# JuliaGenAI/ColBERT.jl

Measured on AMD Instinct MI355X. Metric: queries/sec, top-1000 on 1M-passage corpus, higher is better.
Workload: dtype f32

## Files before the change

colbert.jl_amd/csrc/approx_kernels.hpp:

```cpp
#pragma once
#include <hip/hip_fp16.h>

#include <algorithm>

#include "common.hpp"
#include "search_kernels.hpp"

namespace clb {

typedef __bf16 bf16x8 __attribute__((ext_vector_type(8)));
typedef uint32_t u32x4 __attribute__((ext_vector_type(4)));
typedef uint32_t u32x4_a4 __attribute__((ext_vector_type(4), aligned(4)));
typedef float f32x4_a4 __attribute__((ext_vector_type(4), aligned(4)));

constexpr float kEpsSafety = 1.25f;

inline bool approx_supported(int dim, int nbits) { return dim == kDim && nbits == 2; }
inline size_t approx_cells_bytes(int64_t B, int64_t K, int64_t ) { return (size_t)B * K * 16 * 4 + 2048; }

__device__ __forceinline__ uint32_t f32_to_bf16_rne(float f) {
    const uint32_t u = __float_as_uint(f);
    return (u + 0x7fffu + ((u >> 16) & 1u)) >> 16;
}
__device__ __forceinline__ uint32_t pack_bf16(float lo, float hi) {
// ... 769 lines not shown
            }
            topn_insert<2>(tv, ti, a, id);
        }
        }
    } else {
        for (int c = lane; c < K; c += 64) {
            const float* cr = C + (size_t)c * kDim;
            float a = 0.f;
            for (int d = 0; d < kDim; ++d) a = fmaf(cr[d], qs[d], a);
            topn_insert<2>(tv, ti, a, c);
        }
        if (lane == 0) atomicAdd(&redo_flag[b], 1);
    }
#pragma unroll
    for (int o = 32; o > 0; o >>= 1) {
        const float v0 = __shfl_xor(tv[0], o, 64), v1 = __shfl_xor(tv[1], o, 64);
        const int i0 = __shfl_xor(ti[0], o, 64), i1 = __shfl_xor(ti[1], o, 64);
        topn_insert<2>(tv, ti, v0, i0);
        topn_insert<2>(tv, ti, v1, i1);
    }
    if (lane == 0) {
        sel[((size_t)b * 32 + t) * 2] = ti[0];
        sel[((size_t)b * 32 + t) * 2 + 1] = ti[1] == 0x7fffffff ? ti[0] : ti[1];
    }
}

static __global__ __launch_bounds__(256) void cells_to_half_kernel(const float* __restrict__ cells,
                                                                  uint32_t* __restrict__ cells16, int K) {
    const int b = blockIdx.y;
    const float* src = cells + (size_t)b * K * 32;
    uint32_t* dst = cells16 + (size_t)b * K * 16;
    const int64_t total = (int64_t)K * 16;
    for (int64_t i = (int64_t)blockIdx.x * 256 + threadIdx.x; i < total; i += (int64_t)gridDim.x * 256) {
        const int64_t c = i >> 4;
        const int t = (int)(i & 15);
        const float lo = src[c * 32 + 2 * t], hi = src[c * 32 + 2 * t + 1];
        const __half2 h = __floats2half2_rn(lo, hi);
        dst[i] = *reinterpret_cast<const uint32_t*>(&h);
    }
}

typedef _Float16 f16x8 __attribute__((ext_vector_type(8)));

struct StepTag {
    int j;
    int rows;
    int last;
    int base;
    int g;
    int jh;
    int rowsh;
    int baseh;
};

constexpr int kStepRows = 32;
constexpr uint32_t kPackSpan = (1u << 27) - kStepRows;

__device__ __forceinline__ uint32_t f32_to_f16_floor(float x) {
    const __half hr = __float2half_rn(x);
    uint32_t bits = *reinterpret_cast<const uint16_t*>(&hr);
    if (__half2float(hr) > x) bits = (bits & 0x8000u) ? bits + 1u : (bits == 0u ? 0x8001u : bits - 1u);
    return bits;
}

template <int N>
__device__ __forceinline__ uint32_t lut_offset(uint32_t R, uint32_t lane8) {
    return __builtin_amdgcn_perm(R, lane8, 0x0c0c0000u | ((4u + N) << 8));
}

#define CLB_DPP_F(V, CTRL) __builtin_bit_cast(float, __builtin_amdgcn_update_dpp(0, __builtin_bit_cast(int, (V)), (CTRL), 0xf, 0xf, true))
__device__ __forceinline__ float sum_lanes_0_31(float s) {
    s += CLB_DPP_F(s, 0xB1);
    s += CLB_DPP_F(s, 0x4E);
    s += CLB_DPP_F(s, 0x141);
    s += CLB_DPP_F(s, 0x140);
    const float below = __builtin_bit_cast(float, __builtin_amdgcn_update_dpp(0, __builtin_bit_cast(int, s), 0x142, 0xa, 0xf, false));
    return s + below;
}
__device__ __forceinline__ float max_lane_halves(float m) { return fmaxf(m, __shfl_xor(m, 32, 64)); }

constexpr int kApproxThreads = 768;
constexpr int kApproxLdsLut = 256 * 256;

template <bool ROWS, int GL = 0, bool CELL8 = false>
static __global__ __launch_bounds__(kApproxThreads, kApproxThreads / 256) void score_approx32_kernel(
    const float* __restrict__ weights, const uint32_t* __restrict__ codeinv, const uint8_t* __restrict__ residuals,
    int cbits, float inv_lo, float inv_step, const float* __restrict__ Q, const uint32_t* __restrict__ cells16,
    const uint2* __restrict__ cand_hdr, const int* __restrict__ ncand, float* __restrict__ scores, int K, int T,
    int B, size_t cand_cap, uint16_t* __restrict__ tokmax, const int* __restrict__ list,
    const int* __restrict__ nlist, const float* __restrict__ eps_pair, unsigned long long* __restrict__ rowmask,
    const float4* __restrict__ tscale = nullptr) {
    const uint32_t cmask = (1u << cbits) - 1u;
    const int lane = threadIdx.x & 63;
    const int r = lane & 31, h = lane >> 5;
    const int x = blockIdx.x & 7;
    const int wg = blockIdx.x >> 3;
    const int wg_per_group = gridDim.x >> 3;
    const int wave = __builtin_amdgcn_readfirstlane(threadIdx.x >> 6);
    __shared__ __attribute__((aligned(16))) unsigned char lut_s[kApproxLdsLut];
    __shared__ __attribute__((aligned(16))) float invx[kApproxThreads / 64][2 * kStepRows];
    constexpr int kSlotBytes = CELL8 ? 1024 : 2048;
    constexpr int kRingBytes = 3 * kSlotBytes;
    __shared__ __attribute__((aligned(16))) unsigned char ring_s[GL ? (kApproxThreads / 64) * kRingBytes : 16];
    constexpr int kStageBytes = 16 * 64 + 64;
    __shared__ __attribute__((aligned(16))) unsigned char stage_s[ROWS ? 16 : (kApproxThreads / 64) * kStageBytes];
    unsigned char* mystage = stage_s + (ROWS ? 0 : wave * kStageBytes);
    __shared__ uint32_t mask_s[ROWS ? (kApproxThreads / 64) * 32 : 1];
    uint32_t* mymask = mask_s + (ROWS ? wave * 32 : 0);
    if (ROWS && threadIdx.x < (kApproxThreads / 64) * 32) mask_s[threadIdx.x] = 0u;
    for (int i = threadIdx.x; i < 256 * 32; i += kApproxThreads) {
        const int v = i >> 5;
        *reinterpret_cast<uint2*>(lut_s + (size_t)i * 8) =
            make_uint2(pack_f16(weights[v & 3], weights[(v >> 2) & 3]), pack_f16(weights[(v >> 4) & 3], weights[(v >> 6) & 3]));
    }
    __syncthreads();
    const char* lut = reinterpret_cast<const char*>(lut_s);
    float* myinv = invx[wave];
    const uint32_t lane8 = 8u * (uint32_t)r;
    unsigned char* myring = ring_s + (GL ? wave * kRingBytes : 0);
    const uint32_t ring_lds = (uint32_t)(uintptr_t)(__attribute__((address_space(3))) unsigned char*)myring;
    const uint32_t gl_poff = 16u * (((uint32_t)lane - (((uint32_t)lane >> 4) & 3u)) & 3u);
    const int gl_src0 = (int)((uint32_t)lane & ~3u);
    const int gl_src1 = gl_src0 + 64;
    const uint32_t gl_rot = ((uint32_t)r >> 2) & 3u;
    const uint32_t gl_x0 = (uint32_t)r * 64u + 16u * (((uint32_t)h + gl_rot) & 3u);
    const uint32_t gl_x1 = (uint32_t)r * 64u + 16u * (((uint32_t)h + 2u + gl_rot) & 3u);
    const int gl8_src = (int)(((uint32_t)lane >> 1) << 2);
    const uint32_t gl8_poff = 16u * (((uint32_t)lane ^ ((uint32_t)lane >> 4)) & 1u);
    const uint32_t gl8_x = (uint32_t)r * 32u + 16u * (((uint32_t)h ^ ((uint32_t)r >> 3)) & 1u);

    f16x8 sel1, sel2;
#pragma unroll
    for (int j = 0; j < 8; ++j) {
        sel1[j] = (r == (CELL8 ? 16 * h + j : 8 * h + j)) ? (_Float16)1.0f : (_Float16)0.0f;
        sel2[j] = (r == (CELL8 ? 16 * h + 8 + j : 16 + 8 * h + j)) ? (_Float16)1.0f : (_Float16)0.0f;
    }

    int b_first, b_step, sub, nsub;
    if (B >= 8) { b_first = x; b_step = 8; sub = 0; nsub = 1; }
    else { b_first = x % B; b_step = B * 8 ; sub = x / B; nsub = (8 - b_first + B - 1) / B; }
    const bool grid2d = gridDim.y > 1;
    const int wg_count = grid2d ? (int)gridDim.x : wg_per_group;
    const int wg_index = grid2d ? (int)blockIdx.x : wg;
    if (grid2d) { b_first = blockIdx.y; b_step = B; sub = 0; nsub = 1; }

    for (int b = b_first; b < B; b += b_step) {
        u32x4 qb[8];
        const float4 ts = CELL8 ? tscale[(size_t)b * 32 + r] : make_float4(1.f, 1.f, 0.f, 0.f);
        const float stp = ts.x;
        const float acc_init = CELL8 ? ts.z - 1024.0f : 0.f;
        {
            const float* qrow = Q + ((size_t)b * T + (r < T ? r : T - 1)) * kDim + 64 * h;
#pragma unroll
            for (int s = 0; s < 8; ++s) {
                float4 lo = *reinterpret_cast<const float4*>(qrow + 8 * s);
                float4 hi = *reinterpret_cast<const float4*>(qrow + 8 * s + 4);
                if (r >= T) { lo = make_float4(0.f, 0.f, 0.f, 0.f); hi = lo; }
                if (CELL8) {
                    lo.x *= ts.y; lo.y *= ts.y; lo.z *= ts.y; lo.w *= ts.y;
                    hi.x *= ts.y; hi.y *= ts.y; hi.z *= ts.y; hi.w *= ts.y;
                }
                qb[s] = u32x4{pack_f16(lo.x, lo.y), pack_f16(lo.z, lo.w), pack_f16(hi.x, hi.y), pack_f16(hi.z, hi.w)};
            }
        }
        const uint2* hdr = cand_hdr + (size_t)b * cand_cap;
        const char* c16 = reinterpret_cast<const char*>(cells16 + (size_t)b * K * (CELL8 ? 8 : 16));
        const uint32_t h16 = 16u * (uint32_t)h;
        float* out = scores + (size_t)b * cand_cap;
        uint16_t* tmax = tokmax + (size_t)b * cand_cap * 32 + r;
        const int* lst = ROWS ? list + (size_t)b * cand_cap : nullptr;
        unsigned long long* rmask = ROWS ? rowmask + (size_t)b * cand_cap * 8 : nullptr;
        const float window = ROWS ? 2.f * eps_pair[b] : 0.f;
        const int n = ROWS ? nlist[b] : ncand[b];
        const int n_waves = wg_count * (kApproxThreads / 64) * nsub;
        const int my_wave = (sub * wg_count + wg_index) * (kApproxThreads / 64) + wave;
        const int per_wave = (n + n_waves - 1) / n_waves;
        const int j_first = min(n, my_wave * per_wave), j_end = min(n, j_first + per_wave);

        for (int j0 = j_first; j0 < j_end; j0 += 64) {
        const int jl = j0 + lane;
        int slot_l = jl < j_end ? jl : j0;
        if (ROWS) slot_l = lst[slot_l];
        const uint2 hv = hdr[slot_l];
        const int nd = j_end - j0 < 64 ? j_end - j0 : 64;
        int it_k = 0;
        uint32_t it_off = __builtin_amdgcn_readlane(hv.x, 0);
        int it_len = (int)__builtin_amdgcn_readlane(hv.y, 0);
        int it_slot = __builtin_amdgcn_readlane(slot_l, 0);
        int it_base = 0;

#define CLB_STAGE_A(RB, CV, PM, TAG)                                                                    \
    {                                                                                                       \
        const bool live = it_k < nd;                                                                        \
        const uint32_t e0 = live ? it_off + (uint32_t)it_base : 0u;                                         \
        const int left = live ? it_len - it_base : kStepRows;                                               \
        const int rows = left < kStepRows ? left : kStepRows;                                               \
        int slot_t = live ? it_slot : 0;                                                                    \
        uint32_t d_ = 0;                                                                                    \
        TAG.j = live ? j0 + it_k : -1;                                                                      \
        TAG.rows = rows;                                                                                    \
        TAG.last = 0;                                                                                       \
        TAG.base = it_base;                                                                                 \
        TAG.g = 0; TAG.jh = -1; TAG.rowsh = rows; TAG.baseh = 0;                                            \
        if (left <= kStepRows) {                                        \
            const int kb = it_k + 1;                                                                        \
            const int kk = kb < 64 ? kb : 63;                                                               \
            const uint32_t off_b = __builtin_amdgcn_readlane(hv.x, kk);                                     \
            const int len_b = (int)__builtin_amdgcn_readlane(hv.y, kk);                                     \
            const int slot_b = __builtin_amdgcn_readlane(slot_l, kk);                                       \
            const int gq = (rows + 7) >> 3;                                                                 \
            d_ = off_b - e0;                     \
            if (!ROWS && gq >= 1 && gq < 4 && kb < nd && len_b > 0 && d_ < kPackSpan) {    \
                const int cap = kStepRows - 8 * gq;                                                         \
                TAG.g = gq; TAG.jh = TAG.j; TAG.rowsh = rows; TAG.baseh = it_base;                          \
                TAG.j = j0 + kb; TAG.rows = len_b < cap ? len_b : cap; TAG.base = 0;                         \
                slot_t = slot_b;                                                                            \
                if (len_b <= cap) {                                           \
                    TAG.last = kb + 1 >= nd ? 3 : 1;                                                        \
                    it_k = kb + 1;                                                                          \
                    const int kc = it_k < 64 ? it_k : 63;                                                   \
                    it_off = __builtin_amdgcn_readlane(hv.x, kc);                                           \
                    it_len = (int)__builtin_amdgcn_readlane(hv.y, kc);                                      \
                    it_slot = __builtin_amdgcn_readlane(slot_l, kc);                                        \
                    it_base = 0;                                                                            \
                } else {                                                                                    \
                    it_k = kb; it_off = off_b; it_len = len_b; it_slot = slot_b; it_base = cap;             \
                }                                                                                           \
            } else {                                                                                        \
                d_ = 0;                                                                                     \
                TAG.last = kb >= nd ? 3 : 1;                                                                \
                it_k = kb; it_off = off_b; it_len = len_b; it_slot = slot_b; it_base = 0;                   \
            }                                                                                               \
        } else it_base += kStepRows;                                                                        \
        if (ROWS) PM = tmax[(size_t)slot_t * 32];               \
        const uint32_t q8_ = 8u * (uint32_t)TAG.g;                                                          \
                       \
        const uint32_t rr = (uint32_t)r < q8_ ? min((uint32_t)r, (uint32_t)(TAG.rowsh - 1))                 \
                                              : min((uint32_t)r, q8_ + (uint32_t)(TAG.rows - 1)) + (d_ - q8_); \
         \
        const uint8_t* rbase_ = residuals + (size_t)e0 * 32;                                                \
        const char* cbase_ = reinterpret_cast<const char*>(codeinv + (size_t)e0);                           \
        const uint32_t roff_ = rr * 32u + h16;                                                              \
        const uint32_t coff_ = rr * 4u;                                                                     \
         \
         \
        RB = __builtin_nontemporal_load(reinterpret_cast<const u32x4*>(rbase_ + roff_));                    \
        CV = __builtin_nontemporal_load(reinterpret_cast<const uint32_t*>(cbase_ + coff_));    \
    }
#define CLB_STAGE_G(CV, X0, X1, SLOT)                                                                       \
    if (GL && CELL8) {                                                                                      \
        const uint32_t ca_ = (uint32_t)__builtin_amdgcn_ds_bpermute(gl8_src, (int)CV) & cmask;              \
        asm volatile("s_mov_b32 m0, %1\n\tglobal_load_lds_dwordx4 %0, off"                                  \
                     :: "v"(c16 + ((ca_ << 5) + gl8_poff)), "s"(ring_lds + (SLOT) * 1024u) : "memory");     \
    } else if (GL) {                                                                                        \
        const uint32_t ca_ = (uint32_t)__builtin_amdgcn_ds_bpermute(gl_src0, (int)CV) & cmask;              \
        const uint32_t cb_ = (uint32_t)__builtin_amdgcn_ds_bpermute(gl_src1, (int)CV) & cmask;              \
         \
        asm volatile("s_mov_b32 m0, %2\n\tglobal_load_lds_dwordx4 %0, off\n\t"                            \
                     "s_add_u32 m0, m0, 0x400\n\tglobal_load_lds_dwordx4 %1, off"                          \
                     :: "v"(c16 + ((ca_ << 6) + gl_poff)), "v"(c16 + ((cb_ << 6) + gl_poff)),               \
                        "s"(ring_lds + (SLOT) * 2048u) : "memory", "scc");                                   \
    } else {                                                                                                \
        const char* row_ = CELL8 ? c16 + (((CV & cmask) << 5) + h16) : c16 + (((CV & cmask) << 6) + h16);   \
        if (CELL8) X0 = *reinterpret_cast<const u32x4*>(row_);       \
        else {                                                                                              \
        X0 = *reinterpret_cast<const u32x4*>(row_);                                                         \
        X1 = *reinterpret_cast<const u32x4*>(row_ + 32);                                                    \
        }                                                                                                   \
    }
#define CLB_LUT(W, N) (*reinterpret_cast<const uint2*>(lut + lut_offset<N>(W, lane8)))
#define CLB_STAGE_CM(RB, CV, X0, X1, SLOT, ACC)                                                       \
    {                                                                                                       \
        if (GL && CELL8) {                                                                                  \
             \
            asm volatile("s_waitcnt vmcnt(3)" ::: "memory");                                                \
            X0 = *reinterpret_cast<const u32x4*>(myring + (SLOT) * 1024 + gl8_x);                           \
        } else if (GL) {                                                                                    \
             \
            asm volatile("s_waitcnt vmcnt(4)" ::: "memory");                                                \
            X0 = *reinterpret_cast<const u32x4*>(myring + (SLOT) * 2048 + gl_x0);                           \
            X1 = *reinterpret_cast<const u32x4*>(myring + (SLOT) * 2048 + gl_x1);                           \
        }                                                                                                   \
         \
        __builtin_amdgcn_wave_barrier();                                                                    \
        myinv[r] = fmaf((float)(CV >> cbits), inv_step, inv_lo);                                            \
        __builtin_amdgcn_wave_barrier();                                                                    \
         \
         \
         \
        uint2 tl[16];                                                                                       \
        tl[0] = CLB_LUT(RB[0], 0); tl[1] = CLB_LUT(RB[0], 1); tl[2] = CLB_LUT(RB[0], 2); tl[3] = CLB_LUT(RB[0], 3);         \
        tl[4] = CLB_LUT(RB[1], 0); tl[5] = CLB_LUT(RB[1], 1); tl[6] = CLB_LUT(RB[1], 2); tl[7] = CLB_LUT(RB[1], 3);         \
        tl[8] = CLB_LUT(RB[2], 0); tl[9] = CLB_LUT(RB[2], 1); tl[10] = CLB_LUT(RB[2], 2); tl[11] = CLB_LUT(RB[2], 3);       \
        tl[12] = CLB_LUT(RB[3], 0); tl[13] = CLB_LUT(RB[3], 1); tl[14] = CLB_LUT(RB[3], 2); tl[15] = CLB_LUT(RB[3], 3);     \
        __builtin_amdgcn_sched_barrier(0);                                                                  \
        _Pragma("unroll") for (int i = 0; i < 16; ++i) ACC[i] = acc_init;                                   \
        if (CELL8) {                     \
            const u32x4 raw_ = X0;                                                                          \
            X0 = u32x4{__builtin_amdgcn_perm(0x64646464u, raw_[0], 0x04010400u), __builtin_amdgcn_perm(0x64646464u, raw_[0], 0x04030402u), \
                       __builtin_amdgcn_perm(0x64646464u, raw_[1], 0x04010400u), __builtin_amdgcn_perm(0x64646464u, raw_[1], 0x04030402u)}; \
            X1 = u32x4{__builtin_amdgcn_perm(0x64646464u, raw_[2], 0x04010400u), __builtin_amdgcn_perm(0x64646464u, raw_[2], 0x04030402u), \
                       __builtin_amdgcn_perm(0x64646464u, raw_[3], 0x04010400u), __builtin_amdgcn_perm(0x64646464u, raw_[3], 0x04030402u)}; \
        }                                                                                                   \
        ACC = __builtin_amdgcn_mfma_f32_32x32x16_f16(__builtin_bit_cast(f16x8, X0), sel1, ACC, 0, 0, 0);    \
        ACC = __builtin_amdgcn_mfma_f32_32x32x16_f16(__builtin_bit_cast(f16x8, X1), sel2, ACC, 0, 0, 0);    \
        _Pragma("unroll") for (int s_ = 0; s_ < 8; ++s_)                                                    \
            ACC = __builtin_amdgcn_mfma_f32_32x32x16_f16(                                                   \
                __builtin_bit_cast(f16x8, u32x4{tl[2 * s_].x, tl[2 * s_].y, tl[2 * s_ + 1].x, tl[2 * s_ + 1].y}), \
                __builtin_bit_cast(f16x8, qb[s_]), ACC, 0, 0, 0);                                           \
    }
#define CLB_PASSAGE_END(MX, J, LAST)                                                                        \
    {                                                                                                       \
        float m_ = max_lane_halves(MX);                                                                     \
        if (CELL8) m_ *= stp;                         \
        const float sum = sum_lanes_0_31(r < T ? m_ : 0.f);                      \
        if ((J) >= 0) {                                                                                \
                   \
            const int p_ = ((J) - j0) & 15;                                                                 \
            if (h == 0) *reinterpret_cast<uint16_t*>(mystage + p_ * 64 + 2 * r) = (uint16_t)f32_to_f16_floor(m_); \
            if (lane == 16) *reinterpret_cast<float*>(mystage + 1024 + 4 * p_) = sum;                       \
            if (p_ == 15 || (LAST) == 3) {     \
                const int jb_ = (J) - p_;                                                                   \
                __builtin_amdgcn_wave_barrier();                                                            \
                const u32x4 tk_ = *reinterpret_cast<const u32x4*>(mystage + 16 * lane);                     \
                const float sc_ = *reinterpret_cast<const float*>(mystage + 1024 + 4 * (lane & 15));         \
                if (lane < 4 * (p_ + 1))                                                                    \
                    *reinterpret_cast<u32x4*>(reinterpret_cast<unsigned char*>(tokmax + ((size_t)b * cand_cap + jb_) * 32) + 16 * lane) = tk_; \
                if (lane <= p_) out[jb_ + lane] = sc_;                                                      \
                __builtin_amdgcn_wave_barrier();                                                            \
            }                                                                                               \
        }                                                                                                   \
    }
#define CLB_STAGE_E(ACC, PM, TAG)                                                                     \
    {                                                                                                       \
        f32x4 iq[4];                                                                                        \
        _Pragma("unroll") for (int q = 0; q < 4; ++q)                                                       \
            iq[q] = *reinterpret_cast<const f32x4*>(myinv + 8 * q + 4 * h);                                 \
         \
         \
         \
        float v[16];                                                                                        \
        _Pragma("unroll") for (int i = 0; i < 16; ++i) { v[i] = ACC[i] * iq[i >> 2][i & 3]; asm volatile("" : "+v"(v[i])); } \
        if (ROWS) {                                                                                         \
            const __half pmh = *reinterpret_cast<const __half*>(&PM);                                       \
            const float lo = r < T ? __half2float(pmh) - window : __builtin_inff();    \
             \
             \
             \
            uint32_t lm = 0;                                                                                \
            _Pragma("unroll") for (int i = 0; i < 16; ++i) lm |= !((CELL8 ? v[i] * stp : v[i]) < lo) ? (1u << i) : 0u; \
            lm |= (uint32_t)__builtin_amdgcn_update_dpp(0, (int)lm, 0xB1, 0xf, 0xf, true);         \
            lm |= (uint32_t)__builtin_amdgcn_update_dpp(0, (int)lm, 0x4E, 0xf, 0xf, true);         \
            lm |= (uint32_t)__builtin_amdgcn_update_dpp(0, (int)lm, 0x141, 0xf, 0xf, true);    \
            lm |= (uint32_t)__builtin_amdgcn_update_dpp(0, (int)lm, 0x140, 0xf, 0xf, true);      \
             \
             \
             \
             \
            uint32_t sp_ = ((lm & 0xFu) | ((lm & 0xF0u) << 4) | ((lm & 0xF00u) << 8) | ((lm & 0xF000u) << 12)) << (4 * h); \
            sp_ &= TAG.rows < kStepRows ? (1u << TAG.rows) - 1u : 0xffffffffu;                              \
             \
             \
             \
             \
             \
            const int wd_ = TAG.base >> 5;                                                                  \
            int ln_ = lane;                                                                                 \
            asm volatile("" : "+v"(ln_));      \
            if ((ln_ & 15) == 0 && wd_ < 8 && TAG.j >= 0) mymask[wd_ + 8 * (((ln_ >> 3) & 2) | (ln_ >> 5))] = sp_; \
            if (TAG.last) {                                                                                 \
                __builtin_amdgcn_wave_barrier();                                                            \
                if (ln_ < 16) {          \
                    const int d_ = (ln_ & 7) + 16 * (ln_ >> 3);                                             \
                    const uint32_t mv_ = mymask[d_] | mymask[d_ + 8];                                       \
                    if (TAG.j >= 0) reinterpret_cast<uint32_t*>(rmask + (size_t)TAG.j * 8)[ln_] = mv_;      \
                    mymask[d_] = 0u;                                                                        \
                    mymask[d_ + 8] = 0u;                                                                    \
                }                                                                                           \
                __builtin_amdgcn_wave_barrier();                                                            \
            }                                                                                               \
        } else {                                                                                            \
            if (TAG.g) {               \
                const float q0_ = fmaxf(fmaxf(fmaxf(v[0], v[1]), v[2]), v[3]);                              \
                const float q1_ = fmaxf(fmaxf(fmaxf(v[4], v[5]), v[6]), v[7]);                              \
                const float q2_ = fmaxf(fmaxf(fmaxf(v[8], v[9]), v[10]), v[11]);                            \
                const float q3_ = fmaxf(fmaxf(fmaxf(v[12], v[13]), v[14]), v[15]);                          \
                const float mh_ = fmaxf(fmaxf(mx, q0_), fmaxf(TAG.g > 1 ? q1_ : kNegInf, TAG.g > 2 ? q2_ : kNegInf)); \
                CLB_PASSAGE_END(mh_, TAG.jh, 1);                                                            \
                mx = fmaxf(fmaxf(TAG.g > 1 ? kNegInf : q1_, TAG.g > 2 ? kNegInf : q2_), q3_);               \
            } else {                                                                                        \
            float m01 = fmaxf(fmaxf(v[0], v[1]), v[2]);                                                     \
            float m23 = fmaxf(fmaxf(v[3], v[4]), v[5]);                                                     \
            float m45 = fmaxf(fmaxf(v[6], v[7]), v[8]);                                                     \
            float m67 = fmaxf(fmaxf(v[9], v[10]), v[11]);                                                   \
            float m89 = fmaxf(fmaxf(v[12], v[13]), v[14]);                                                  \
            m01 = fmaxf(fmaxf(m01, m23), m45);                                                              \
            m67 = fmaxf(fmaxf(m67, m89), v[15]);                                                            \
            mx = fmaxf(fmaxf(mx, m01), m67);                                                                \
            }                                                                                               \
            if (TAG.last) {                                                                                 \
                CLB_PASSAGE_END(mx, TAG.j, TAG.last);                                                       \
                mx = kNegInf;                                                                               \
            }                                                                                               \
        }                                                                                                   \
    }

        float mx = kNegInf;
        u32x4 rb0, rb1, rb2, xa0, xa1, xa2, xb0, xb1, xb2;
        uint32_t cv0, cv1, cv2, cw0, cw1, cw2;
        uint16_t pm0 = 0, pm1 = 0, pm2 = 0;
        StepTag t0, t1, t2;
        f32x16 acc0;
        CLB_STAGE_A(rb0, cv0, pm0, t0);
        CLB_STAGE_A(rb1, cv1, pm1, t1);
        CLB_STAGE_G(cv0, xa0, xb0, 0); cw0 = cv0;
        while (t0.j >= 0) {
            CLB_STAGE_A(rb2, cv2, pm2, t2);
            CLB_STAGE_G(cv1, xa1, xb1, 1); cw1 = cv1;
            CLB_STAGE_CM(rb0, cw0, xa0, xb0, 0, acc0);
            CLB_STAGE_E(acc0, pm0, t0);
            CLB_STAGE_A(rb0, cv0, pm0, t0);
            CLB_STAGE_G(cv2, xa2, xb2, 2); cw2 = cv2;
            CLB_STAGE_CM(rb1, cw1, xa1, xb1, 1, acc0);
            CLB_STAGE_E(acc0, pm1, t1);
            CLB_STAGE_A(rb1, cv1, pm1, t1);
            CLB_STAGE_G(cv0, xa0, xb0, 0); cw0 = cv0;
            CLB_STAGE_CM(rb2, cw2, xa2, xb2, 2, acc0);
            CLB_STAGE_E(acc0, pm2, t2);
        }
        }
#undef CLB_STAGE_A
#undef CLB_STAGE_G
#undef CLB_STAGE_CM
#undef CLB_STAGE_E
#undef CLB_PASSAGE_END
#undef CLB_LUT
    }
}

static __global__ __launch_bounds__(256) void code_adjacency_kernel(const uint32_t* __restrict__ codes0, int64_t n,
                                                                   unsigned long long* __restrict__ count) {
    unsigned long long c = 0;
    for (int64_t i = (int64_t)blockIdx.x * 256 + threadIdx.x + 1; i < n; i += (int64_t)gridDim.x * 256)
        c += (codes0[i] >> 1) == (codes0[i - 1] >> 1);
#pragma unroll
    for (int o = 32; o > 0; o >>= 1) c += __shfl_xor(c, o, 64);
    if ((threadIdx.x & 63) == 0 && c) atomicAdd(count, c);
}

struct ApproxConsts {
    float cn_max;
    float rn_max;
    float inv_max;
    float rb_max;
    float dw_rn;
    float inv_qerr;
    float dc_max;
};

struct QueryBound { float eps_t, eps_sum; bool unsafe; };
__device__ __forceinline__ QueryBound query_bound(const float* __restrict__ Q, int b, int T, const ApproxConsts& ac,
                                                  float* s_qn, float* s_dq, const float4* __restrict__ tscale = nullptr,
                                                  float* s_aux = nullptr ,
                                                  bool cell8 = false) {
    const int tid = threadIdx.x;
    if (tid == 0) { *s_qn = 0.f; *s_dq = 0.f; }
    if (tscale && tid < 4) s_aux[tid] = 0.f;
    __syncthreads();
    {
        const int t = tid >> 5, part = tid & 31;
        float a = 0.f, dd = 0.f, d8 = 0.f;
        if (t < T) {
            const float4 v = *reinterpret_cast<const float4*>(Q + ((size_t)b * T + t) * kDim + 4 * part);
            a = fmaf(v.x, v.x, fmaf(v.y, v.y, fmaf(v.z, v.z, v.w * v.w)));
            const float dx = v.x - round_f16(v.x), dy = v.y - round_f16(v.y);
            const float dz = v.z - round_f16(v.z), dw = v.w - round_f16(v.w);
            dd = fmaf(dx, dx, fmaf(dy, dy, fmaf(dz, dz, dw * dw)));
            if (tscale && cell8) {
                const float4 ts = tscale[(size_t)b * 32 + t];
                const float sx = v.x * ts.y, sy = v.y * ts.y, sz = v.z * ts.y, sw = v.w * ts.y;
                const float ex = sx - round_f16(sx), ey = sy - round_f16(sy), ez = sz - round_f16(sz), ew = sw - round_f16(sw);
                d8 = fmaf(ex, ex, fmaf(ey, ey, fmaf(ez, ez, ew * ew)));
            }
        }
#pragma unroll
        for (int o = 16; o > 0; o >>= 1) { a += __shfl_xor(a, o, 64); dd += __shfl_xor(dd, o, 64); d8 += __shfl_xor(d8, o, 64); }
        if (t < T && part == 0) {
            atomicMax(reinterpret_cast<unsigned int*>(s_qn), __float_as_uint(sqrtf(a) * 1.001f));
            atomicMax(reinterpret_cast<unsigned int*>(s_dq), __float_as_uint(sqrtf(dd) * 1.001f));
            if (tscale) {
                const float4 ts = tscale[(size_t)b * 32 + t];
                atomicMax(reinterpret_cast<unsigned int*>(s_aux), __float_as_uint(ts.x * sqrtf(d8) * 1.001f));
                atomicMax(reinterpret_cast<unsigned int*>(s_aux + 1), __float_as_uint(ts.x));
                atomicMax(reinterpret_cast<unsigned int*>(s_aux + 3), __float_as_uint(ts.w));
                if (!(ts.x > 0.f) || !(sqrtf(a) * ts.y < 3.0e4f)) s_aux[2] = 1.f;
            }
        }
    }
    __syncthreads();
    const float u = 5.9604645e-08f;
    const float qn = *s_qn;
    const float e_cells = kEpsSafety * centroid_product_bound(qn, *s_dq, ac.cn_max, ac.dc_max) + 4.8828125e-04f * qn * ac.cn_max + 2.9802322e-08f;
    float e_qr = 1.001f * (*s_dq * ac.rb_max + qn * ac.dw_rn) + 2.f * 128.f * u * qn * ac.rn_max;
    float e_tab = e_cells;
    bool bad8 = false;
    if (tscale) {
        const float amax = s_aux[2] != 0.f ? qn * ac.cn_max : fminf(s_aux[3] * 1.0001f, qn * ac.cn_max);
        const float e_f16 = kEpsSafety * centroid_product_bound(qn, *s_dq, ac.cn_max, ac.dc_max) + 4.8828125e-04f * amax + 2.9802322e-08f;
        e_tab = e_f16;
        if (cell8) {
            const float dq8 = s_aux[0], step_max = s_aux[1];
// ... 472 lines not shown
```

colbert.jl_amd/csrc/search.hip:

```cpp
#include <algorithm>
#include <atomic>
#include <cstdlib>
#include <cstring>
#include <memory>
#include <numeric>

#include "approx_kernels.hpp"
#include "after_kernels.hpp"
#include "generic_kernels.hpp"
#include "group_kernels.hpp"
#include "index_change_kernels.hpp"
#include "prior_kernels.hpp"
#include "search_kernels.hpp"
#include "sort.hpp"

using namespace clb;

namespace {

enum KernelId {
    KID_CENTROID_SCORES = 0,
    KID_TOPN,
    KID_MARK,
    KID_COMPACT,
    KID_SCORE_EXACT,
    KID_SCORE_APPROX,
    KID_SELECT,
    KID_ROWS,
    KID_TOPK,
    KID_COUNT
};
const char* kKernelNames[KID_COUNT] = {"centroid_scores", "top_nprobe", "mark_candidates", "compact_candidates",
                                       "score_exact",     "score_approx", "select_margin", "rescore_rows",
                                       "topk"};

struct Prof {
    bool on = false;
    bool counters = false;
    std::vector<std::pair<hipEvent_t, hipEvent_t>> pending[KID_COUNT];
    std::vector<hipEvent_t> pool;
    hipEvent_t chain = nullptr;
    hipStream_t chain_stream = nullptr;
    double total_ms[KID_COUNT] = {0};
    int64_t launches[KID_COUNT] = {0};
    bool failed = false;
    hipEvent_t get() {
        if (!pool.empty()) {
            hipEvent_t e = pool.back();
            pool.pop_back();
            return e;
        }
        hipEvent_t e = nullptr;
        if (hipEventCreate(&e) != hipSuccess) { failed = true; return nullptr; }
        return e;
    }
};

}

struct clb_filter {
    uint64_t owner = 0;
    int device = 0;
    int64_t n_docs = 0, count = 0;
    DevBuf bits;
};

struct clb_grouping {
    uint64_t owner = 0;
    int device = 0;
    int64_t n_docs = 0, count = 0;
    DevBuf gid;
};

struct clb_prior {
    uint64_t owner = 0;
    int device = 0;
    int64_t n_docs = 0;
    float max_abs = 0.f;
    DevBuf values;
};

struct Workspace {
    int64_t Bcap = 0, Tcap = 0, npcap = 0, kcap = 0;
    int64_t Ttuned = 0;
    size_t cand_cap = 0;
    int W = 0, nblk_bitmap = 0, topn_blocks = 0;
    bool x1_table = false;
    bool have_range = false;
    bool cell8 = false;
    size_t filt_cap = 0;
    size_t ivf_cap = 0;
    struct { bool valid = false; const float* dQ = nullptr; int64_t T = 0, B = 0, nprobe = 0, k = 0; void* stream = nullptr;
             size_t filt_now = 0; const clb_grouping* grp = nullptr; int64_t group_base = 0;
             const clb_prior* prior = nullptr; float weight = 0.f; } pending;
    struct { bool valid = false; int64_t B = 0, k = 0, generation = 0; const clb_grouping* grp = nullptr; void* stream = nullptr; } grouped_done;
    DevBuf Qdev, cells, cells_q, partial, sel, bitmap, blocksum, ncand, cand, cand_hdr, scores, list, nlist, thresh,
        outp, outs, flags, stats, redo, rowmask, eps_pair, tokmax, tau_glob, wsel, bounds, tscale, rangep, cells8;
    bool grouped = false;
    DevBuf grp_list, grp_n, grp_list2, grp_n2, grp_tau;
    int64_t mcap = 0;
    DevBuf hit_p, hit_s, hit_cut, hit_run, hit_list, hit_n;
    bool prior = false;
    DevBuf prior_tau;
    bool after = false;
    DevBuf after_list, after_n, after_tau, after_cur_s, after_cur_p;
    DevBuf g_cells, g_keys, g_keys2, g_vals, g_vals2, g_scratch, g_sort_tmp;
};

constexpr int kWorkspaceSlots = 4;

struct clb_searcher {
    int device = 0;
    uint64_t serial = 0;
    int64_t dim = 0, K = 0, n_docs = 0, n_emb = 0, pid_offset = 0;
    int nbits = 0;
    int mode = 0;
    int wide_select = -1;
    bool approx_ok = false;
    bool bounds_synced = false;
    bool ivf_sorted = false;
    bool generic = false;
    int64_t max_doclen = 0;
    hipStream_t stream = nullptr;
    DevBuf centroids;
    DevBuf weights;
    DevBuf codes0;
    DevBuf residuals;
    DevBuf doc_off;
    DevBuf live;
    DevBuf ivf_off;
    DevBuf ivf_pid;
    DevBuf codeinv;
    int cbits = 0;
    float inv_lo = 0.f, inv_step = 0.f;
    DevBuf cent_hi, cent_lo;
    DevBuf cent_f16;
    float dc_f16 = 0.f;
    int s1_x1 = -1;
    int gather_lds = 0;
    double code_adjacency = 0.0;
    int cell8 = -1;
    ApproxConsts approx_consts{};
    std::vector<uint32_t> ivf_len_sorted;
    Workspace ws[kWorkspaceSlots];
    Prof prof;
    int64_t last_cand_docs = 0, last_cand_embs = 0, last_resc_docs = 0, last_resc_embs = 0;
    int64_t index_bytes = 0;
    int64_t generation = 0;
};

namespace {

struct Batch {
    const float* dQ = nullptr;
    int B = 0, T = 0, nprobe = 0, k = 0;
    int64_t* d_out_pids = nullptr; float* d_out_scores = nullptr; int64_t* d_n_cand = nullptr;
    const clb_filter* const* filt = nullptr;
    int filt_all = 0;
    size_t filt_now = 0;
    const clb_grouping* grp = nullptr;
    int per_group = 0;
    int64_t* d_hit_pids = nullptr; float* d_hit_scores = nullptr;
    const clb_prior* prior = nullptr;
    float prior_weight = 1.f;
    const float* d_after_s = nullptr; const int64_t* d_after_p = nullptr;
    bool stats_keep = false;
    int phase = 0, n_shards = 0;
    float* d_local_top = nullptr; const float* d_all_top = nullptr;
    int64_t group_base = 0;
    int64_t* d_local_gid = nullptr; const int64_t* d_all_gid = nullptr;
    int64_t* d_out_gids = nullptr; int64_t* d_edge_gids = nullptr;
    float* d_local_mabs = nullptr; const float* d_all_mabs = nullptr;
};
Batch make_batch(const float* dQ, int64_t B, int64_t T, int64_t nprobe, int64_t k) {
    Batch q;
    q.dQ = dQ; q.B = (int)B; q.T = (int)T; q.nprobe = (int)nprobe; q.k = (int)k;
    return q;
}

struct Timed {
    clb_searcher* s;
    int id;
    hipStream_t st;
    hipEvent_t a = nullptr, b = nullptr;
    Timed(clb_searcher* s_, int id_, hipStream_t st_) : s(s_), id(id_), st(st_) {
        if (s->prof.on && id >= 0) {
            if (s->prof.chain && s->prof.chain_stream == st) {
                a = s->prof.chain;
            } else {
                a = s->prof.get();
                if (a && hipEventRecord(a, st) != hipSuccess) { s->prof.pool.push_back(a); a = nullptr; s->prof.failed = true; }
            }
            b = a ? s->prof.get() : nullptr;
        }
    }
    ~Timed() {
        if (!s->prof.on || id < 0) return;
        if (a && b && hipEventRecord(b, st) == hipSuccess) {
            s->prof.pending[id].push_back({a, b});
            s->prof.chain = b;
            s->prof.chain_stream = st;
        } else {
            s->prof.failed = true;
            s->prof.chain = nullptr;
        }
    }
};

inline int token_tiles(int64_t T) { return T <= 32 ? 1 : T <= 64 ? 2 : 4; }
inline int64_t padded_nprobe(int64_t nprobe) { return nprobe <= 2 ? 2 : nprobe <= 8 ? 8 : nprobe <= 32 ? 32 : nprobe; }

inline bool cell8_rows(const clb_searcher* s) { return s->cell8 == 1 && s->approx_ok; }

inline bool single_product_table(const clb_searcher* s) {
    return (s->s1_x1 == 1 || (s->s1_x1 < 0 && s->bounds_synced)) && s->cent_f16.p && s->dc_f16 > 0.f;
}

inline int default_gather_lds(const clb_searcher* s) { return s->code_adjacency < 0.2 && s->K * 64 > ((int64_t)4 << 20); }

void allow_large_topk_lds() {
    allow_dynamic_lds(reinterpret_cast<const void*>(topk_kernel), (int)(sizeof(unsigned long long) * kMaxTopK));
}

constexpr int64_t kSubBatch = 64;

int next_pow2(int x) {
    int p = 1;
    while (p < x) p <<= 1;
    return p;
}

int ensure_workspace_sized(clb_searcher* s, Workspace& w, int64_t B, int64_t T, int64_t nprobe, int64_t k, size_t filt_count,
                           bool grouped, int64_t per_group, bool prior, bool after) {
    const int64_t t_tuned = T <= 128 ? T : 0;
    if (B <= w.Bcap && T <= w.Tcap && t_tuned <= w.Ttuned && nprobe <= w.npcap && k <= w.kcap && filt_count <= w.filt_cap &&
        (!grouped || w.grouped) && per_group <= w.mcap && (!prior || w.prior) && (!after || w.after))
        return CLB_OK;
    CLB_HIP(hipDeviceSynchronize());
    B = std::max(B, w.Bcap); T = std::max(T, w.Tcap);
    nprobe = std::max(nprobe, w.npcap); k = std::max(k, w.kcap);
    per_group = std::max(per_group, w.mcap);
    const int64_t Ttuned = std::max(w.Ttuned, t_tuned);
    const int64_t Tpad = token_tiles(std::max<int64_t>(Ttuned, 1)) * 32;
    size_t lists = (size_t)std::min<int64_t>(T * nprobe, s->K);
    size_t cap = 0;
    for (size_t i = 0; i < lists; ++i) cap += s->ivf_len_sorted[i];
    cap = std::min<size_t>(cap, (size_t)s->n_docs);
    w.ivf_cap = (std::max<size_t>(cap, 1) + 3) & ~(size_t)3;
    cap = std::max<size_t>(cap, std::max(filt_count, w.filt_cap));
    cap = std::max<size_t>(cap, 1);
    w.cand_cap = (cap + 3) & ~(size_t)3;
    w.W = (int)((s->n_docs + 31) / 32);
    w.nblk_bitmap = (w.W + kScanBlock * kWordsPerThread - 1) / (kScanBlock * kWordsPerThread);
    w.topn_blocks = (int)std::max<int64_t>(1, std::min<int64_t>(256, s->K / 512));
    const int64_t NPs = padded_nprobe(nprobe);
    const bool general = s->generic;
    CLB_TRY(w.Qdev.ensure(sizeof(float) * B * T * s->dim));
    const bool general_batched = general && s->dim % 4 == 0 && s->dim <= 256;
    if (Ttuned > 0 && ((!general && !(nprobe <= 2 && Ttuned <= 32)) || general_batched))
        CLB_TRY(w.cells.ensure(sizeof(float) * B * s->K * Tpad));
    if (Ttuned > 0 && (!general || general_batched))
        CLB_TRY(w.partial.ensure(sizeof(ValIdx) * B * w.topn_blocks * Tpad * std::min<int64_t>(NPs, 32)));
    CLB_TRY(w.sel.ensure(sizeof(int) * B * std::max<int64_t>(Tpad, T) * NPs));
    const size_t bm_bytes = sizeof(uint32_t) * (size_t)B * w.W;
    const bool bm_new = bm_bytes > w.bitmap.bytes || !w.bitmap.p;
    CLB_TRY(w.bitmap.ensure(bm_bytes));
    if (bm_new) CLB_HIP(hipMemsetAsync(w.bitmap.p, 0, w.bitmap.bytes, s->stream));
    CLB_TRY(w.blocksum.ensure(sizeof(int) * B * w.nblk_bitmap));
    CLB_TRY(w.ncand.ensure(sizeof(int) * B));
    CLB_TRY(w.cand.ensure(sizeof(uint32_t) * B * w.cand_cap));
    {
        const size_t nsl = ((size_t)w.nblk_bitmap + kMarkSliceBlocks - 1) / kMarkSliceBlocks;
        const size_t nbig = ((size_t)w.nblk_bitmap + kMarkSliceBlocksBig - 1) / kMarkSliceBlocksBig;
        if (nsl > 16) CLB_TRY(w.bounds.ensure(sizeof(uint32_t) * B * T * nprobe * (nbig + 1)));
    }
    CLB_TRY(w.cand_hdr.ensure(sizeof(uint2) * B * w.cand_cap));
    CLB_TRY(w.scores.ensure(sizeof(float) * B * w.cand_cap));
    CLB_TRY(w.list.ensure(sizeof(int) * B * w.cand_cap));
    CLB_TRY(w.nlist.ensure(sizeof(int) * B));
    CLB_TRY(w.thresh.ensure(sizeof(float) * B * 2));
    CLB_TRY(w.outp.ensure(sizeof(int64_t) * B * k * std::max<int64_t>(per_group, 1)));
    CLB_TRY(w.outs.ensure(sizeof(float) * B * k * std::max<int64_t>(per_group, 1)));
    CLB_TRY(w.flags.ensure(sizeof(int) * B));
    if (!w.stats.p) {
        CLB_TRY(w.stats.ensure(sizeof(unsigned long long) * 8));
        CLB_HIP(hipMemset(w.stats.p, 0, sizeof(unsigned long long) * 8));
    }
    if (s->approx_ok && Ttuned > 0) {
        CLB_TRY(w.cells_q.ensure(approx_cells_bytes(B, s->K, Tpad)));
        CLB_TRY(w.rowmask.ensure(sizeof(unsigned long long) * 8 * B * w.cand_cap));
        CLB_TRY(w.eps_pair.ensure(sizeof(float) * B));
        CLB_TRY(w.tokmax.ensure(sizeof(uint16_t) * 32 * B * w.cand_cap));
    }
    if (grouped || w.grouped) {
        CLB_TRY(w.grp_list.ensure(sizeof(int) * B * w.cand_cap));
        CLB_TRY(w.grp_n.ensure(sizeof(int) * B));
        CLB_TRY(w.grp_tau.ensure(sizeof(float) * B));
        if (s->approx_ok) {
            CLB_TRY(w.grp_list2.ensure(sizeof(int) * B * w.cand_cap));
            CLB_TRY(w.grp_n2.ensure(sizeof(int) * B));
        }
        w.grouped = true;
    }
    if (per_group > 0) {
        CLB_TRY(w.hit_p.ensure(sizeof(int64_t) * B * k));
        CLB_TRY(w.hit_s.ensure(sizeof(float) * B * k));
        if (s->approx_ok) {
            CLB_TRY(w.hit_cut.ensure(sizeof(unsigned long long) * B * w.cand_cap));
            CLB_TRY(w.hit_run.ensure(sizeof(int) * B * w.cand_cap));
            CLB_TRY(w.hit_list.ensure(sizeof(int) * B * w.cand_cap));
            CLB_TRY(w.hit_n.ensure(sizeof(int) * B));
        }
    }
    if (prior || w.prior) {
        CLB_TRY(w.prior_tau.ensure(sizeof(float) * 2 * B));
        w.prior = true;
    }
    if (after || w.after) {
        CLB_TRY(w.after_list.ensure(sizeof(int) * B * w.cand_cap));
        CLB_TRY(w.after_n.ensure(sizeof(int) * B));
        CLB_TRY(w.after_tau.ensure(sizeof(float) * B));
        CLB_TRY(w.after_cur_s.ensure(sizeof(float) * B));
        CLB_TRY(w.after_cur_p.ensure(sizeof(int64_t) * B));
        w.after = true;
    }
    w.Bcap = B; w.Tcap = T; w.Ttuned = Ttuned; w.npcap = nprobe; w.kcap = k; w.mcap = per_group;
    w.filt_cap = std::max(w.filt_cap, filt_count);
    CLB_HIP(hipStreamSynchronize(s->stream));
    return CLB_OK;
}

int ensure_workspace(clb_searcher* s, Workspace& w, int64_t B, int64_t T, int64_t nprobe, int64_t k, size_t filt_count = 0,
                     bool grouped = false, int64_t per_group = 0, bool prior = false, bool after = false) {
    const int rc = ensure_workspace_sized(s, w, B, T, nprobe, k, filt_count, grouped, per_group, prior, after);
    if (rc) {
        w.Bcap = 0;
        if (rc == CLB_ENOMEM && filt_count > w.filt_cap)
            return fail(CLB_EUNSUPPORTED, "no room for the candidate buffers of a filter of %zu passages (CLB_FILTER_ALL, %lld "
                                          "queries per pass): %s", filt_count, (long long)B, std::string(last_error()).c_str());
    }
    return rc;
}

template <int NP>
void launch_topn(clb_searcher* s, Workspace& w, hipStream_t st, int B, int Tpad) {
    hipLaunchKernelGGL(topn_partial_kernel<NP>, dim3(w.topn_blocks, B), dim3(256), 0, st,
                       w.cells.as<float>(), w.partial.as<ValIdx>(), (int)s->K, Tpad);
    hipLaunchKernelGGL(topn_final_kernel<NP>, dim3(B), dim3(Tpad), 0, st, w.partial.as<ValIdx>(),
                       w.sel.as<int>(), w.topn_blocks, Tpad);
}

template <int NBITS>
void launch_score_exact(clb_searcher* s, Workspace& w, hipStream_t st, const float* dQ, int B, int T, const int* list,
                        const int* nlist, int grid_x) {
    hipLaunchKernelGGL(score_exact_kernel<NBITS>, dim3(grid_x, B), dim3(256), 0, st, s->centroids.as<float>(),
                       s->weights.as<float>(), s->codes0.as<uint32_t>(), s->residuals.as<uint8_t>(),
                       w.cand_hdr.as<uint2>(), dQ, w.ncand.as<int>(), w.scores.as<float>(), T, w.cand_cap, list,
                       nlist);
}

int select_by_sort(clb_searcher* s, Workspace& w, hipStream_t st, const float* cells, size_t stride_t, size_t stride_c,
                   int T, int nprobe, int NP, int* sel_b);

int select_top_nprobe(clb_searcher* s, Workspace& w, hipStream_t st, int B, int T, int Tpad, int nprobe) {
    const int NPs = (int)padded_nprobe(nprobe);
    if (NPs == 2) launch_topn<2>(s, w, st, B, Tpad);
    else if (NPs == 8) launch_topn<8>(s, w, st, B, Tpad);
    else if (NPs == 32) launch_topn<32>(s, w, st, B, Tpad);
    else
        for (int b = 0; b < B; ++b)
            CLB_TRY(select_by_sort(s, w, st, w.cells.as<float>() + (size_t)b * s->K * Tpad, 1, (size_t)Tpad, T, nprobe, NPs,
                                   w.sel.as<int>() + (size_t)b * Tpad * NPs));
    return CLB_OK;
}

// ... 263 lines not shown
                       w.cand.as<uint32_t>() + (size_t)b0 * w.cand_cap, w.ncand.as<int>() + b0,
                       list ? list + (size_t)b0 * w.cand_cap : nullptr, list ? nlist + b0 : nullptr, q.d_after_s + b0,
                       q.d_after_p + b0, w.cand_cap, s->pid_offset, w.after_list.as<int>() + (size_t)b0 * w.cand_cap,
                       w.after_n.as<int>() + b0);
}

int topk_of(clb_searcher* s, Workspace& w, hipStream_t st, const Batch& q, int b0, int n) {
    launch_boost(w, st, q, b0, n, nullptr, nullptr, nullptr);
    if (q.d_after_s) {
        launch_after(s, w, st, q, b0, n, nullptr, nullptr);
        return launch_topk(s, w, st, q, b0, n, w.after_list.as<int>(), w.after_n.as<int>(), 0);
    }
    if (!q.grp) return launch_topk(s, w, st, q, b0, n, nullptr, nullptr, 0);
    launch_collapse(w, st, q, b0, n, nullptr, nullptr, w.grp_list.as<int>(), w.grp_n.as<int>());
    CLB_TRY(launch_topk(s, w, st, q, b0, n, w.grp_list.as<int>(), w.grp_n.as<int>(), 0));
    launch_hits(s, w, st, q, b0, n, nullptr, nullptr);
    return CLB_OK;
}

int run_retrieve_general(clb_searcher* s, Workspace& w, hipStream_t st, const Batch& q, int b) {
    const int T = q.T, nprobe = q.nprobe;
    CLB_TRY(w.g_cells.ensure(sizeof(float) * (size_t)T * s->K));
    hipLaunchKernelGGL(generic_cells_kernel, dim3((unsigned)((s->K + 127) / 128), T), dim3(128), sizeof(float) * s->dim, st,
                       s->centroids.as<float>(), q.dQ + (size_t)b * T * s->dim, (int)s->dim, (int)s->K, w.g_cells.as<float>());
    CLB_TRY(select_by_sort(s, w, st, w.g_cells.as<float>(), (size_t)s->K, 1, T, nprobe, nprobe, w.sel.as<int>()));
    return mark_and_compact(s, w, st, q, b, 1, T, nprobe, false);
}

bool general_batched_ok(const clb_searcher* s, int T) { return s->dim % 4 == 0 && s->dim <= 256 && T <= 128; }

int run_retrieve_general_batched(clb_searcher* s, Workspace& w, hipStream_t st, const Batch& q) {
    const int Tpad = token_tiles(q.T) * 32;
    auto cells_kernel = s->dim <= 128 ? generic_cells_mfma_kernel<32> : generic_cells_mfma_kernel<64>;
    hipLaunchKernelGGL(cells_kernel, dim3((unsigned)((s->K + 63) / 64), (unsigned)q.B), dim3(256), 0, st, s->centroids.as<float>(),
                       q.dQ, (int)s->dim, (int)s->K, q.T, Tpad, w.cells.as<float>());
    CLB_TRY(select_top_nprobe(s, w, st, q.B, q.T, Tpad, q.nprobe));
    return mark_and_compact(s, w, st, q, 0, q.B, Tpad, (int)padded_nprobe(q.nprobe), true);
}

int run_search_general(clb_searcher* s, Workspace& w, hipStream_t st, const Batch& q) {
    const float* dQ = q.dQ;
    const int B = q.B, T = q.T;
    s->prof.chain = nullptr;
    if (general_batched_ok(s, T)) {
        CLB_TRY(run_retrieve_general_batched(s, w, st, q));
        const dim3 grid((unsigned)std::max(64, 2048 / std::max(1, B)), (unsigned)B);
        const size_t lds = sizeof(float) * (((size_t)1 << s->nbits) + (size_t)T * (s->dim + 1));
        if (lds > 64 * 1024) {
            allow_dynamic_lds(reinterpret_cast<const void*>(generic_score_mfma_fast_kernel<32>), (int)lds);
            allow_dynamic_lds(reinterpret_cast<const void*>(generic_score_mfma_fast_kernel<64>), (int)lds);
        }
        auto score_kernel = s->dim <= 128 ? generic_score_mfma_fast_kernel<32> : generic_score_mfma_fast_kernel<64>;
        hipLaunchKernelGGL(score_kernel, grid, dim3(256), lds, st, s->centroids.as<float>(), s->weights.as<float>(),
                           s->codes0.as<uint32_t>(), s->residuals.as<uint8_t>(), w.cand_hdr.as<uint2>(), w.ncand.as<int>(), dQ,
                           (int)s->dim, s->nbits, T, w.cand_cap, w.scores.as<float>());
        CLB_HIP(hipGetLastError());
        return topk_of(s, w, st, q, 0, B);
    }
    const int grid = 1024;
    const size_t max_len = (size_t)std::max<int64_t>(s->max_doclen, 1);
    CLB_TRY(w.g_scratch.ensure(sizeof(float) * grid * max_len * s->dim));
    for (int b = 0; b < B; ++b) {
        CLB_TRY(run_retrieve_general(s, w, st, q, b));
        if (T <= 16 * kGenericMaxTokenGroups && s->dim % 4 == 0)
            hipLaunchKernelGGL(generic_score_mfma_kernel, dim3(grid), dim3(256), sizeof(float) * ((size_t)1 << s->nbits), st,
                               s->centroids.as<float>(), s->weights.as<float>(), s->codes0.as<uint32_t>(),
                               s->residuals.as<uint8_t>(), w.cand_hdr.as<uint2>() + (size_t)b * w.cand_cap,
                               w.ncand.as<int>() + b, dQ + (size_t)b * T * s->dim, (int)s->dim, s->nbits, T,
                               w.scores.as<float>() + (size_t)b * w.cand_cap);
        else
            hipLaunchKernelGGL(generic_score_kernel, dim3(grid), dim3(256), sizeof(float) * T, st, s->centroids.as<float>(),
                               s->weights.as<float>(), s->codes0.as<uint32_t>(), s->residuals.as<uint8_t>(),
                               w.cand_hdr.as<uint2>() + (size_t)b * w.cand_cap, w.ncand.as<int>() + b,
                               dQ + (size_t)b * T * s->dim, (int)s->dim, s->nbits, T, w.g_scratch.as<float>(), max_len,
                               w.scores.as<float>() + (size_t)b * w.cand_cap);
        CLB_HIP(hipGetLastError());
        CLB_TRY(topk_of(s, w, st, q, b, 1));
    }
    return CLB_OK;
}

constexpr size_t kWideSelectCap = 131072;

void launch_pass1(clb_searcher* s, Workspace& w, hipStream_t st, const float* dQ, dim3 grid, int B, int T) {
    auto kern = w.cell8 ? (s->gather_lds ? score_approx32_kernel<false, 1, true> : score_approx32_kernel<false, 0, true>)
                        : (s->gather_lds ? score_approx32_kernel<false, 1, false> : score_approx32_kernel<false, 0, false>);
    hipLaunchKernelGGL(kern, grid, dim3(kApproxThreads), 0, st, s->weights.as<float>(),
                       s->codeinv.as<uint32_t>(), s->residuals.as<uint8_t>(), s->cbits, s->inv_lo, s->inv_step, dQ,
                       w.cell8 ? w.cells8.as<uint32_t>() : w.cells_q.as<uint32_t>(), w.cand_hdr.as<uint2>(), w.ncand.as<int>(),
                       w.scores.as<float>(), (int)s->K, T, B, w.cand_cap, w.tokmax.as<uint16_t>(), (const int*)nullptr,
                       (const int*)nullptr, (const float*)nullptr, (unsigned long long*)nullptr,
                       (const float4*)w.tscale.as<float4>());
}
inline float bound_dc(const clb_searcher* s, const Workspace& w) {
    return (w.x1_table || (s->bounds_synced && s->s1_x1 != 0 && s->cent_f16.p)) ? s->dc_f16 : 0.f;
}
int launch_select(clb_searcher* s, Workspace& w, hipStream_t st, const Batch& q, const float* tau_in, bool coarse_tau = false) {
    const float* dQ = q.dQ;
    const int B = q.B, T = q.T, k = q.k;
    const size_t most = std::max(w.ivf_cap, q.filt_now);
    const bool wide = s->wide_select == 1 || (s->wide_select < 0 && most >= kWideSelectCap);
    if (!wide) {
        ApproxConsts ac = s->approx_consts;
        ac.dc_max = bound_dc(s, w);
        hipLaunchKernelGGL(select_margin_kernel, dim3(B), dim3(1024), 0, st, w.scores.as<float>(), w.ncand.as<int>(), dQ, T, k,
                           w.cand_cap, ac, w.list.as<int>(), w.nlist.as<int>(), w.thresh.as<float>(),
                           w.eps_pair.as<float>(), tau_in, coarse_tau ? 1 : 0,
                           w.have_range ? (const float4*)w.tscale.as<float4>() : (const float4*)nullptr, w.cell8 ? 1 : 0);
        return CLB_OK;
    }
    CLB_TRY(w.wsel.ensure(sizeof(WideSel) * B));
    CLB_HIP(hipMemsetAsync(w.wsel.p, 0, sizeof(WideSel) * B, st));
    const dim3 grid(kWideBlocks, B);
    ApproxConsts acw = s->approx_consts;
    acw.dc_max = bound_dc(s, w);
    hipLaunchKernelGGL(wide_minmax_kernel, grid, dim3(1024), 0, st, w.scores.as<float>(), w.ncand.as<int>(), dQ, T, w.cand_cap,
                       acw, w.wsel.as<WideSel>(), w.eps_pair.as<float>(),
                       w.have_range ? (const float4*)w.tscale.as<float4>() : (const float4*)nullptr, w.cell8 ? 1 : 0);
    if (!tau_in)
        for (int pass = 0; pass < 4; ++pass)
            hipLaunchKernelGGL(wide_hist_kernel, grid, dim3(1024), 0, st, w.scores.as<float>(), w.ncand.as<int>(), k, w.cand_cap,
                               w.wsel.as<WideSel>(), pass);
    hipLaunchKernelGGL(wide_count_kernel, grid, dim3(1024), 0, st, w.scores.as<float>(), w.ncand.as<int>(), k, w.cand_cap,
                       w.wsel.as<WideSel>(), tau_in);
    hipLaunchKernelGGL(wide_emit_kernel, grid, dim3(1024), 0, st, w.scores.as<float>(), w.ncand.as<int>(), k, w.cand_cap,
                       (const WideSel*)w.wsel.as<WideSel>(), tau_in, w.list.as<int>(), w.nlist.as<int>(), w.thresh.as<float>());
    return CLB_OK;
}

int run_search(clb_searcher* s, Workspace& w, hipStream_t st, const Batch& q) {
    const float* dQ = q.dQ;
    const int B = q.B, T = q.T, k = q.k, phase = q.phase;
    const bool two_pass = s->mode == 1 && s->approx_ok && T <= 32;
    if (phase != 0 && !two_pass) return fail(CLB_EUNSUPPORTED, "the two-phase sharded search needs the two-pass mode");
    if (s->generic || T > 128) return run_search_general(s, w, st, q);
    s->prof.chain = nullptr;
    if (phase == 2) {
        CLB_TRY(w.tau_glob.ensure(sizeof(float) * B));
        if (q.prior) {
            ApproxConsts ac = s->approx_consts;
            ac.dc_max = bound_dc(s, w);
            hipLaunchKernelGGL(prior_global_tau_kernel, dim3(B), dim3(1024), 0, st, q.d_all_top, q.d_all_gid, q.d_all_mabs,
                               q.n_shards, B, k, (const float*)nullptr, dQ, T, ac,
                               w.have_range ? (const float4*)w.tscale.as<float4>() : (const float4*)nullptr, w.cell8 ? 1 : 0,
                               w.tau_glob.as<float>());
        } else if (q.grp)
            hipLaunchKernelGGL(group_global_tau_kernel, dim3(B), dim3(1024), 0, st, q.d_all_top, q.d_all_gid, q.n_shards, B, k,
                               w.tau_glob.as<float>());
        else
            hipLaunchKernelGGL(global_tau_kernel, dim3(B), dim3(1024), 0, st, q.d_all_top, q.n_shards, B, k, w.tau_glob.as<float>());
        Timed t(s, KID_SELECT, st);
        CLB_TRY(launch_select(s, w, st, q, (const float*)w.tau_glob.as<float>()));
    } else {
        CLB_TRY(run_retrieve(s, w, st, q));
        if (s->prof.counters) {
            if (!q.stats_keep) CLB_HIP(hipMemsetAsync(w.stats.p, 0, sizeof(unsigned long long) * 8, st));
            s->prof.chain = nullptr;
        }
        if (two_pass) {
            {
                Timed t(s, KID_SCORE_APPROX, st);
                constexpr int kWgPerGroup = 32;
                const double est_cand = 0.5 * T * q.nprobe * (double)s->n_emb / (double)std::max<int64_t>(1, s->K);
                const int gxq = est_cand < 6000.0 ? std::max(8, 256 / B) : 0;
                const dim3 approx_grid = gxq > 0 && B > 1 ? dim3(gxq, B) : dim3(8 * kWgPerGroup);
                launch_pass1(s, w, st, dQ, approx_grid, B, T);
            }
            if (q.prior && phase == 0) {
                Timed t(s, KID_SELECT, st);
                float* ptau = w.prior_tau.as<float>();
                float* mabs = ptau + w.Bcap;
                launch_boost(w, st, q, 0, B, nullptr, nullptr, mabs);
                if (q.grp) launch_collapse(w, st, q, 0, B, nullptr, nullptr, w.grp_list.as<int>(), w.grp_n.as<int>());
                ApproxConsts ac = s->approx_consts;
                ac.dc_max = bound_dc(s, w);
                hipLaunchKernelGGL(prior_tau_kernel, dim3(B), dim3(1024), 0, st, w.scores.as<float>(), w.ncand.as<int>(),
                                   q.grp ? (const int*)w.grp_list.as<int>() : (const int*)nullptr,
                                   q.grp ? (const int*)w.grp_n.as<int>() : (const int*)nullptr, k, w.cand_cap, (const float*)mabs,
                                   dQ, T, ac, w.have_range ? (const float4*)w.tscale.as<float4>() : (const float4*)nullptr,
                                   w.cell8 ? 1 : 0, ptau);
                CLB_TRY(launch_select(s, w, st, q, (const float*)ptau));
            } else if (q.d_after_s) {
                Timed t(s, KID_SELECT, st);
                ApproxConsts ac = s->approx_consts;
                ac.dc_max = bound_dc(s, w);
                hipLaunchKernelGGL(after_cut_kernel, dim3(B), dim3(1024), 0, st, w.scores.as<float>(), w.ncand.as<int>(), k,
                                   w.cand_cap, q.d_after_s, dQ, T, ac,
                                   w.have_range ? (const float4*)w.tscale.as<float4>() : (const float4*)nullptr, w.cell8 ? 1 : 0,
                                   w.after_tau.as<float>());
                CLB_TRY(launch_select(s, w, st, q, (const float*)w.after_tau.as<float>()));
            } else {
                Timed t(s, KID_SELECT, st);
                if (phase == 1) launch_boost(w, st, q, 0, B, nullptr, nullptr, q.d_local_mabs);
                if (q.grp && phase == 1) {
                    launch_collapse(w, st, q, 0, B, nullptr, nullptr, w.grp_list.as<int>(), w.grp_n.as<int>());
                    hipLaunchKernelGGL(group_local_top_kernel, dim3(B), dim3(1024), 0, st, w.scores.as<float>(),
                                       w.cand.as<uint32_t>(), w.grp_list.as<int>(), w.grp_n.as<int>(), q.grp->gid.as<uint32_t>(),
                                       q.group_base, k, w.cand_cap, q.d_local_top, q.d_local_gid);
                    CLB_HIP(hipGetLastError());
                    return CLB_OK;
                }
                if (q.grp) {
                    launch_collapse(w, st, q, 0, B, nullptr, nullptr, w.grp_list.as<int>(), w.grp_n.as<int>());
                    hipLaunchKernelGGL(group_tau_kernel, dim3(B), dim3(1024), 0, st, w.scores.as<float>(), w.grp_list.as<int>(),
                                       w.grp_n.as<int>(), k, w.cand_cap, w.grp_tau.as<float>());
                    CLB_TRY(launch_select(s, w, st, q, (const float*)w.grp_tau.as<float>()));
                    if (q.per_group > 0)
                        hipLaunchKernelGGL(group_extend_kernel, dim3(B), dim3(1024), 0, st, w.scores.as<float>(),
                                           w.cand.as<uint32_t>(), w.ncand.as<int>(), q.grp->gid.as<uint32_t>(),
                                           w.thresh.as<float>(), q.per_group, w.cand_cap, w.hit_cut.as<unsigned long long>(),
                                           w.hit_run.as<int>(), w.hit_list.as<int>(), w.hit_n.as<int>());
                } else
                    CLB_TRY(launch_select(s, w, st, q, nullptr, phase == 0));
            }
        }
    }
    const bool extended = two_pass && q.grp && q.per_group > 0 && phase == 0;
    const int* list = two_pass ? (extended ? w.hit_list.as<int>() : w.list.as<int>()) : nullptr;
    const int* nlist = two_pass ? (extended ? w.hit_n.as<int>() : w.nlist.as<int>()) : nullptr;
    if (phase == 1) {
        hipLaunchKernelGGL(local_top_kernel, dim3(B), dim3(1024), 0, st, w.scores.as<float>(), list, nlist,
                           w.thresh.as<float>(), k, w.cand_cap, q.d_local_top);
        CLB_HIP(hipGetLastError());
        return CLB_OK;
    }
    const bool subset = list != nullptr;
    if (subset) {
        Timed t(s, KID_ROWS, st);
        constexpr int kRowsGx = 256;
        const dim3 rows_grid = B > 1 ? dim3(std::max(1, kRowsGx / B), B) : dim3(8 * 32);
        auto rows_kernel = w.cell8 ? score_approx32_kernel<true, 0, true> : score_approx32_kernel<true, 0, false>;
        hipLaunchKernelGGL(rows_kernel, rows_grid, dim3(kApproxThreads), 0, st, s->weights.as<float>(),
                           s->codeinv.as<uint32_t>(), s->residuals.as<uint8_t>(), s->cbits, s->inv_lo, s->inv_step, dQ,
                           w.cell8 ? w.cells8.as<uint32_t>() : w.cells_q.as<uint32_t>(), w.cand_hdr.as<uint2>(), w.ncand.as<int>(),
                           w.scores.as<float>(), (int)s->K, T, B, w.cand_cap, w.tokmax.as<uint16_t>(), list, nlist,
                           w.eps_pair.as<float>(), w.rowmask.as<unsigned long long>(), (const float4*)w.tscale.as<float4>());
    }
    {
        Timed t(s, KID_SCORE_EXACT, st);
        const int gx = list ? std::max(1, 1024 / B) : std::max(1, 2048 / B);
        constexpr int kFlatGx = 768;
        if (subset)
            hipLaunchKernelGGL(score_exact_flat_kernel, dim3(std::max(1, kFlatGx / B), B), dim3(256), 0, st, s->centroids.as<float>(),
                               s->weights.as<float>(), s->codes0.as<uint32_t>(), s->residuals.as<uint8_t>(),
                               w.cand_hdr.as<uint2>(), dQ, w.scores.as<float>(), T, w.cand_cap, list, nlist,
                               w.rowmask.as<unsigned long long>());
        else
            switch (s->nbits) {
                case 1: launch_score_exact<1>(s, w, st, dQ, B, T, list, nlist, gx); break;
                case 2: launch_score_exact<2>(s, w, st, dQ, B, T, list, nlist, gx); break;
                case 4: launch_score_exact<4>(s, w, st, dQ, B, T, list, nlist, gx); break;
                default: return fail(CLB_EUNSUPPORTED, "nbits=%d not supported by the HIP search path", s->nbits);
            }
    }
    const int* tlist = list;
    const int* tnlist = nlist;
    auto collapse_exact = [&]() {
        launch_boost(w, st, q, 0, B, list, nlist, nullptr);
        if (q.d_after_s) {
            launch_after(s, w, st, q, 0, B, list, nlist);
            tlist = w.after_list.as<int>(); tnlist = w.after_n.as<int>();
        }
        if (!q.grp) return;
        int* gl = list ? w.grp_list2.as<int>() : w.grp_list.as<int>();
        int* gn = list ? w.grp_n2.as<int>() : w.grp_n.as<int>();
        launch_collapse(w, st, q, 0, B, list, nlist, gl, gn);
        tlist = gl; tnlist = gn;
    };
    if (k <= kMaxTopK) {
        Timed t(s, KID_TOPK, st);
        collapse_exact();
        const int ranked = tlist != nullptr;
        if (ranked)
            hipLaunchKernelGGL(topk_rank_kernel, dim3(kRankBlocks, B), dim3(1024), 0, st, w.scores.as<float>(),
                               w.cand.as<uint32_t>(), reported_count(w, q), tlist, tnlist, k, w.cand_cap, s->pid_offset,
                               q.d_out_pids, q.d_out_scores, w.flags.as<int>(), q.d_n_cand);
        CLB_TRY(launch_topk(s, w, st, q, 0, B, tlist, tnlist, ranked));
    } else {
        s->prof.chain = nullptr;
        collapse_exact();
        CLB_TRY(launch_topk(s, w, st, q, 0, B, tlist, tnlist, 0));
    }
    if (q.grp) launch_hits(s, w, st, q, 0, B, list, nlist);
    if (q.grp && q.d_out_gids) launch_result_groups(s, w, st, q.grp, q.group_base, q.d_out_pids, B, k, q.d_out_gids, q.d_edge_gids);
    if (s->prof.counters) {
        hipLaunchKernelGGL(batch_stats_kernel, dim3(32, B), dim3(256), 0, st, w.cand.as<uint32_t>(),
                           w.ncand.as<int>(), list, nlist, s->doc_off.as<uint32_t>(), w.cand_cap,
                           w.stats.as<unsigned long long>(),
                           subset ? w.rowmask.as<unsigned long long>() : (const unsigned long long*)nullptr, T);
    }
    CLB_HIP(hipGetLastError());
    return CLB_OK;
}

int check_filters(const clb_searcher* s, const clb_filter* const* filters, int64_t B, int scope, size_t* filt_count) {
    *filt_count = 0;
    if (scope != CLB_FILTER_CANDIDATES && scope != CLB_FILTER_ALL)
        return fail(CLB_EARGUMENT, "scope must be CLB_FILTER_CANDIDATES (0) or CLB_FILTER_ALL (1), got %d", scope);
    if (!filters) return CLB_OK;
    for (int64_t b = 0; b < B; ++b) {
        const clb_filter* f = filters[b];
        if (!f) continue;
        if (f->owner != s->serial)
            return fail(CLB_EARGUMENT, "the filter of query %lld was made for another searcher", (long long)b);
        if (f->n_docs != s->n_docs)
            return fail(CLB_EARGUMENT, "the filter of query %lld: filter made before an append; make another", (long long)b);
        if (scope == CLB_FILTER_ALL) *filt_count = std::max(*filt_count, (size_t)f->count);
    }
    return CLB_OK;
}

int check_prior(const clb_searcher* s, const clb_prior* p, float weight) {
    if (!p) return CLB_OK;
    if (!std::isfinite(weight)) return fail(CLB_EARGUMENT, "prior_weight must be finite, got %g", (double)weight);
    if (p->owner != s->serial) return fail(CLB_EARGUMENT, "the prior was made for another searcher");
    if (p->n_docs != s->n_docs)
        return fail(CLB_EARGUMENT, "prior made before an append; make another");
    if (!(std::fabs((double)weight) * (double)p->max_abs < (double)FLT_MAX))
        return fail(CLB_EARGUMENT, "prior_weight %g times the prior's largest |value| %g is not below FLT_MAX", (double)weight,
// ... 73 lines not shown
    o->off[n] = (uint32_t)o->total;
    return -1;
}
int passage_offsets(const int64_t* doclens, int64_t n, int64_t n_emb, const char* noun, Offsets* o) {
    const int64_t bad = running_offsets(doclens, n, o);
    if (bad >= 0) return fail(CLB_EARGUMENT, "negative doclen at %s %lld", noun, (long long)(bad + 1));
    if (o->total != n_emb)
        return fail(CLB_EDIMENSION, "sum(doclens)=%lld must equal the number of embeddings %lld", (long long)o->total, (long long)n_emb);
    return CLB_OK;
}

template <class T>
struct DevWord {
    DevBuf buf;
    T value{};
    T* ptr() const { return buf.as<T>(); }
    int init(hipStream_t st) {
        CLB_TRY(buf.alloc(sizeof(T)));
        CLB_HIP(hipMemsetAsync(buf.p, 0, sizeof(T), st));
        return CLB_OK;
    }
    int read(hipStream_t st) {
        CLB_HIP(hipMemcpyAsync(&value, buf.p, sizeof(T), hipMemcpyDeviceToHost, st));
        CLB_HIP(hipStreamSynchronize(st));
        CLB_HIP(hipGetLastError());
        return CLB_OK;
    }
};
enum { kErrIvfId = 1, kErrCode = 2, kErrUnsortedList = 4 };

int stage_codes(hipStream_t st, const uint32_t* codes, hipMemcpyKind kind, int64_t n, int64_t K, uint32_t* dst, int* err) {
    if (n == 0) return CLB_OK;
    CLB_HIP(hipMemcpyAsync(dst, codes, sizeof(uint32_t) * n, kind, st));
    hipLaunchKernelGGL(codes_to_zero_based_kernel, dim3((unsigned)((n + 255) / 256)), dim3(256), 0, st, dst, n, (uint32_t)K, err);
    return CLB_OK;
}
int bad_codes() { return fail(CLB_EDOMAIN, "All the codes must be in the valid range of centroid IDs!"); }

int alloc_padded_rows(hipStream_t st, int64_t n, size_t row_bytes, DevBuf* codes, DevBuf* res) {
    CLB_TRY(codes->alloc(sizeof(uint32_t) * (n + kStepRows)));
    CLB_TRY(res->alloc(row_bytes * (n + kStepRows)));
    CLB_HIP(hipMemsetAsync(codes->as<uint32_t>() + n, 0, sizeof(uint32_t) * kStepRows, st));
    CLB_HIP(hipMemsetAsync(res->as<uint8_t>() + row_bytes * n, 0, row_bytes * kStepRows, st));
    return CLB_OK;
}

int order_rows_by_code(hipStream_t st, const uint32_t* codes_src, const uint32_t* offsets_dev, int64_t n_emb, int64_t n_docs,
                       const uint8_t* res_src, size_t row_bytes, uint32_t* codes_dst, uint8_t* res_dst) {
    DevBuf keys, keys2, vals, perm;
    CLB_TRY(keys.alloc(sizeof(uint64_t) * n_emb));
    CLB_TRY(keys2.alloc(sizeof(uint64_t) * n_emb));
    CLB_TRY(vals.alloc(sizeof(uint32_t) * n_emb));
    CLB_TRY(perm.alloc(sizeof(uint32_t) * n_emb));
    const dim3 blocks((unsigned)((n_emb + 255) / 256));
    hipLaunchKernelGGL(passage_code_keys_kernel, blocks, dim3(256), 0, st, codes_src, offsets_dev, n_emb, (int)n_docs,
                       keys.as<unsigned long long>(), vals.as<uint32_t>());
    CLB_TRY(sort_pairs_u64(keys.as<uint64_t>(), keys2.as<uint64_t>(), vals.as<uint32_t>(), perm.as<uint32_t>(), (size_t)n_emb, st));
    hipLaunchKernelGGL(permute_codes_kernel, blocks, dim3(256), 0, st, perm.as<uint32_t>(), codes_src, codes_dst, n_emb);
    const int pieces = (int)(row_bytes / 16);
    hipLaunchKernelGGL(permute_rows16_kernel, dim3((unsigned)((n_emb * pieces + 255) / 256)), dim3(256), 0, st, perm.as<uint32_t>(),
                       reinterpret_cast<const uint4*>(res_src), reinterpret_cast<uint4*>(res_dst), n_emb, pieces);
    CLB_HIP(hipGetLastError());
    CLB_HIP(hipStreamSynchronize(st));
    return CLB_OK;
}

int build_live_bitmap(hipStream_t st, const uint32_t* doc_off, int64_t n_docs, DevBuf* live) {
    const int64_t W = (n_docs + 31) / 32;
    CLB_TRY(live->alloc(sizeof(uint32_t) * (size_t)W));
    if (W > 0) hipLaunchKernelGGL(passage_live_kernel, dim3((unsigned)((W + 255) / 256)), dim3(256), 0, st, doc_off, (int)n_docs,
                                  live->as<uint32_t>());
    return CLB_OK;
}

std::vector<uint32_t> sorted_list_lengths(const std::vector<uint32_t>& ivf_off) {
    std::vector<uint32_t> len(ivf_off.size() - 1);
    for (size_t c = 0; c + 1 < ivf_off.size(); ++c) len[c] = ivf_off[c + 1] - ivf_off[c];
    std::sort(len.begin(), len.end(), std::greater<uint32_t>());
    return len;
}

int64_t resident_bytes(const clb_searcher* s) {
    return (int64_t)(s->centroids.bytes + s->weights.bytes + s->codes0.bytes + s->residuals.bytes + s->doc_off.bytes +
                     s->ivf_off.bytes + s->ivf_pid.bytes + s->codeinv.bytes + s->live.bytes);
}

struct IndexTables {
    double code_adjacency = 0.0;
    ApproxConsts consts{};
    float inv_lo = 0.f, inv_step = 0.f;
    DevBuf codeinv;
};

int derive_index_tables(const clb_searcher* s, const uint32_t* codes0, const uint8_t* residuals, int64_t n_emb, IndexTables* t) {
    {
        DevWord<unsigned long long> adj;
        const int64_t n_sample = std::min<int64_t>(n_emb, (int64_t)1 << 24);
        CLB_TRY(adj.init(s->stream));
        if (n_sample > 1)
            hipLaunchKernelGGL(code_adjacency_kernel, dim3(1024), dim3(256), 0, s->stream, codes0, n_sample, adj.ptr());
        CLB_TRY(adj.read(s->stream));
        t->code_adjacency = n_sample > 1 ? (double)adj.value / (double)(n_sample - 1) : 0.0;
    }
    if (s->approx_ok) {
        CLB_TRY(t->codeinv.alloc(sizeof(uint32_t) * (n_emb + kStepRows)));
        CLB_HIP(hipMemsetAsync(t->codeinv.p, 0, t->codeinv.bytes, s->stream));
    }
    return build_approx_tables(s->stream, s->centroids.as<float>(), s->weights.as<float>(), codes0, residuals, n_emb, (int)s->K,
                               s->approx_ok ? t->codeinv.as<uint32_t>() : nullptr, s->cbits, 1 << s->nbits, &t->consts,
                               &t->inv_lo, &t->inv_step);
}

inline void swap_buf(DevBuf& a, DevBuf& b) { std::swap(a.p, b.p); std::swap(a.bytes, b.bytes); }

constexpr float ApproxConsts::* kBoundConsts[6] = {&ApproxConsts::cn_max, &ApproxConsts::rn_max, &ApproxConsts::inv_max,
                                                   &ApproxConsts::rb_max, &ApproxConsts::dw_rn,  &ApproxConsts::inv_qerr};
void bound_consts_to_abi(const ApproxConsts& a, float* c) { for (int i = 0; i < 6; ++i) c[i] = a.*kBoundConsts[i]; }
void raise_bound_consts(ApproxConsts& a, const float* c) {
    for (int i = 0; i < 6; ++i) a.*kBoundConsts[i] = std::max(a.*kBoundConsts[i], c[i]);
}

void install_index_tables(clb_searcher* s, IndexTables& t, bool keep_max = false) {
    s->code_adjacency = t.code_adjacency;
    s->gather_lds = default_gather_lds(s);
    swap_buf(s->codeinv, t.codeinv);
    s->inv_lo = t.inv_lo; s->inv_step = t.inv_step;
    float old[6];
    bound_consts_to_abi(s->approx_consts, old);
    s->approx_consts = t.consts;
    s->dc_f16 = std::isfinite(s->approx_consts.dc_max) ? s->approx_consts.dc_max : 0.f;
    s->approx_consts.dc_max = 0.f;
    if (keep_max) raise_bound_consts(s->approx_consts, old);
    s->index_bytes = resident_bytes(s);
}

struct IndexChange {
    DevBuf codes0, residuals, doc_off, live, ivf_off, ivf_pid;
    IndexTables tables;
    std::vector<uint32_t> h_ivf_off;
    int64_t n_docs = 0, n_emb = 0, max_doclen = 0;
};

int begin_index_change(const clb_searcher* s) {
    CLB_TRY(use_device(s->device));
    CLB_HIP(hipDeviceSynchronize());
    return CLB_OK;
}

int check_pid_range(const clb_searcher* s, const int64_t* pids, int64_t n) {
    for (int64_t i = 0; i < n; ++i)
        if (pids[i] <= s->pid_offset || pids[i] > s->pid_offset + s->n_docs)
            return fail(CLB_EBOUNDS, "pid %lld (entry %lld) outside %lld..%lld", (long long)pids[i], (long long)i,
                        (long long)(s->pid_offset + 1), (long long)(s->pid_offset + s->n_docs));
    return CLB_OK;
}

int stage_new_rows(const clb_searcher* s, const uint32_t* codes_in, const uint32_t* off_dev, int64_t n_emb, int64_t n,
                   const uint8_t* residuals, bool on_device, uint32_t* codes_dst, uint8_t* res_dst) {
    const hipStream_t st = s->stream;
    const hipMemcpyKind kind = on_device ? hipMemcpyDeviceToDevice : hipMemcpyHostToDevice;
    const size_t rows = (size_t)(s->dim / 8 * s->nbits);
    if (s->generic) {
        CLB_HIP(hipMemcpyAsync(codes_dst, codes_in, sizeof(uint32_t) * n_emb, hipMemcpyDeviceToDevice, st));
        CLB_HIP(hipMemcpyAsync(res_dst, residuals, rows * n_emb, kind, st));
        return CLB_OK;
    }
    DevBuf res_in;
    if (!on_device || ((uintptr_t)residuals & 15)) {
        CLB_TRY(res_in.alloc(rows * n_emb));
        CLB_HIP(hipMemcpyAsync(res_in.p, residuals, rows * n_emb, kind, st));
        residuals = res_in.as<uint8_t>();
    }
    return order_rows_by_code(st, codes_in, off_dev, n_emb, n, residuals, rows, codes_dst, res_dst);
}

int mark_passages(const clb_searcher* s, const int64_t* pids, int64_t n, DevBuf* d_pids, DevBuf* bits, int* err) {
    CLB_TRY(upload(*d_pids, pids, sizeof(int64_t) * n, s->stream));
    CLB_TRY(bits->alloc(sizeof(uint32_t) * (size_t)((s->n_docs + 31) / 32)));
    CLB_HIP(hipMemsetAsync(bits->p, 0, bits->bytes, s->stream));
    hipLaunchKernelGGL(filter_mark_kernel<false>, dim3((unsigned)((n + 255) / 256)), dim3(256), 0, s->stream, d_pids->as<int64_t>(), n,
                       s->pid_offset, (int)s->n_docs, bits->as<uint32_t>(), err);
    return CLB_OK;
}

int scan_kept_entries(const clb_searcher* s, const uint32_t* named, DevBuf* pos) {
    DevBuf flag;
    CLB_TRY(flag.alloc(sizeof(uint32_t) * (s->n_emb + 1)));
    CLB_TRY(pos->alloc(sizeof(uint32_t) * (s->n_emb + 1)));
    hipLaunchKernelGGL(ivf_keep_flags_kernel, dim3((unsigned)((s->n_emb + 1 + 255) / 256)), dim3(256), 0, s->stream,
                       s->ivf_pid.as<uint32_t>(), named, s->n_emb, flag.as<uint32_t>());
    return exclusive_scan_u32(flag.as<uint32_t>(), pos->as<uint32_t>(), (size_t)s->n_emb, s->stream);
}

int compact_lists(const clb_searcher* s, const DevBuf& pos, int64_t n_kept, DevBuf* off, DevBuf* pid) {
    CLB_TRY(off->alloc(sizeof(uint32_t) * (s->K + 1)));
    CLB_TRY(pid->alloc(sizeof(uint32_t) * n_kept));
    hipLaunchKernelGGL(ivf_compact_kernel, dim3((unsigned)((s->n_emb + 1 + 255) / 256)), dim3(256), 0, s->stream,
                       s->ivf_pid.as<uint32_t>(), pos.as<uint32_t>(), s->n_emb, pid->as<uint32_t>());
    hipLaunchKernelGGL((list_offsets_kernel<true, false>), dim3((unsigned)((s->K + 1 + 255) / 256)), dim3(256), 0, s->stream,
                       s->ivf_off.as<uint32_t>(), pos.as<uint32_t>(), (const uint32_t*)nullptr, (int)(s->K + 1), off->as<uint32_t>());
    return CLB_OK;
}

struct NewEntries {
    DevBuf off, code, pid;
};
int sort_new_entries(const clb_searcher* s, const uint32_t* codes_in, const uint32_t* off_dev, int64_t n, const int64_t* d_pids,
                     int64_t pid_base, int64_t n_emb, bool by_pid, NewEntries* e) {
    const hipStream_t st = s->stream;
    DevBuf hist, pid_in, pid2, code2;
    CLB_TRY(hist.alloc(sizeof(uint32_t) * (s->K + 1)));
    CLB_TRY(pid_in.alloc(sizeof(uint32_t) * n_emb));
    CLB_TRY(e->off.alloc(sizeof(uint32_t) * (s->K + 1)));
    CLB_TRY(e->code.alloc(sizeof(uint32_t) * n_emb));
    CLB_TRY(e->pid.alloc(sizeof(uint32_t) * n_emb));
    CLB_HIP(hipMemsetAsync(hist.p, 0, hist.bytes, st));
    if (n_emb > 0)
        hipLaunchKernelGGL(hist_pid_kernel, dim3((unsigned)((n_emb + 255) / 256)), dim3(256), 0, st, codes_in, off_dev, d_pids,
                           s->pid_offset, (uint32_t)pid_base, n_emb, (int)n, hist.as<uint32_t>(), pid_in.as<uint32_t>());
    CLB_TRY(exclusive_scan_u32(hist.as<uint32_t>(), e->off.as<uint32_t>(), (size_t)s->K, st));
    int pid_bits = 1, code_bits = 1;
    while (((int64_t)1 << pid_bits) < s->n_docs) ++pid_bits;
    while (((int64_t)1 << code_bits) < s->K) ++code_bits;
    const uint32_t *codes = codes_in, *pids = pid_in.as<uint32_t>();
    if (by_pid) {
        CLB_TRY(pid2.alloc(sizeof(uint32_t) * n_emb));
        CLB_TRY(code2.alloc(sizeof(uint32_t) * n_emb));
        CLB_TRY(sort_pairs_u32(pids, pid2.as<uint32_t>(), codes, code2.as<uint32_t>(), (size_t)n_emb, pid_bits, st));
        codes = code2.as<uint32_t>(); pids = pid2.as<uint32_t>();
    }
    return sort_pairs_u32(codes, e->code.as<uint32_t>(), pids, e->pid.as<uint32_t>(), (size_t)n_emb, code_bits, st);
}

int merge_lists(const clb_searcher* s, const uint32_t* old_off, const uint32_t* old_pid, const NewEntries& e, IndexChange* c) {
    CLB_TRY(c->ivf_off.alloc(sizeof(uint32_t) * (s->K + 1)));
    CLB_TRY(c->ivf_pid.alloc(sizeof(uint32_t) * c->n_emb));
    hipLaunchKernelGGL((list_offsets_kernel<false, true>), dim3((unsigned)((s->K + 1 + 255) / 256)), dim3(256), 0, s->stream, old_off,
                       (const uint32_t*)nullptr, e.off.as<uint32_t>(), (int)(s->K + 1), c->ivf_off.as<uint32_t>());
    const int64_t tiles = (c->n_emb + kTile - 1) / kTile;
    if (tiles > 0)
        hipLaunchKernelGGL(ivf_merge_kernel, dim3((unsigned)std::min<int64_t>(tiles, 8192)), dim3(256), 0, s->stream, old_off,
                           e.off.as<uint32_t>(), c->ivf_off.as<uint32_t>(), old_pid, e.pid.as<uint32_t>(), (int)s->K, c->n_emb,
                           c->ivf_pid.as<uint32_t>());
    return CLB_OK;
}

template <class F>
void with_piece(size_t row_bytes, F&& f) {
    if (row_bytes % 16 == 0) f(uint4{});
    else if (row_bytes % 4 == 0) f(uint32_t{});
    else f(uint8_t{});
}

int commit_index_change(clb_searcher* s, IndexChange& c) {
    const hipStream_t st = s->stream;
    CLB_HIP(hipGetLastError());
    c.h_ivf_off.resize((size_t)s->K + 1);
    CLB_HIP(hipMemcpyAsync(c.h_ivf_off.data(), c.ivf_off.p, sizeof(uint32_t) * (s->K + 1), hipMemcpyDeviceToHost, st));
    CLB_HIP(hipStreamSynchronize(st));
    if ((int64_t)c.h_ivf_off[s->K] != c.n_emb)
        return fail(CLB_EHIP, "the changed inverted lists hold %lld entries, expected %lld", (long long)c.h_ivf_off[s->K],
                    (long long)c.n_emb);
    if (!s->generic) CLB_TRY(derive_index_tables(s, c.codes0.as<uint32_t>(), c.residuals.as<uint8_t>(), c.n_emb, &c.tables));
    CLB_HIP(hipStreamSynchronize(st));
    CLB_HIP(hipGetLastError());

    swap_buf(s->codes0, c.codes0); swap_buf(s->residuals, c.residuals); swap_buf(s->doc_off, c.doc_off);
    swap_buf(s->ivf_off, c.ivf_off); swap_buf(s->ivf_pid, c.ivf_pid); swap_buf(s->live, c.live);
    s->n_docs = c.n_docs; s->n_emb = c.n_emb; s->max_doclen = c.max_doclen;
    s->ivf_len_sorted = sorted_list_lengths(c.h_ivf_off);
    if (s->generic) s->index_bytes = resident_bytes(s);
    else install_index_tables(s, c.tables, s->bounds_synced);
    for (auto& w : s->ws) {
        w.Bcap = 0;
        w.filt_cap = 0;
        w.bitmap.release();
        w.pending.valid = false;
    }
    ++s->generation;
    return CLB_OK;
}

int replace_passages(clb_searcher* s, int64_t n, const int64_t* pids, const Offsets* add, const uint32_t* codes,
                     const uint8_t* residuals, bool on_device, int64_t* n_changed) {
    const int64_t n_old = s->n_emb, n_docs = s->n_docs, K = s->K, n_add = add ? add->total : 0;
    const bool staged = n_add > 0;
    CLB_TRY(begin_index_change(s));
    const hipStream_t st = s->stream;
    const size_t rows = (size_t)(s->dim / 8 * s->nbits);
    IndexChange c;
    DevWord<ChangeCounts> counts;
    {
        DevBuf codes_in, d_pids, stage_off, named, slot, len;
        DevWord<int> err;
        CLB_TRY(err.init(st));
        CLB_TRY(counts.init(st));
        CLB_TRY(mark_passages(s, pids, n, &d_pids, &named, err.ptr()));
        if (staged) {
            CLB_TRY(codes_in.alloc(sizeof(uint32_t) * n_add));
            CLB_TRY(stage_codes(st, codes, on_device ? hipMemcpyDeviceToDevice : hipMemcpyHostToDevice, n_add, K,
                                codes_in.as<uint32_t>(), err.ptr()));
            CLB_TRY(upload(stage_off, add->off.data(), sizeof(uint32_t) * add->off.size(), st));
            CLB_TRY(slot.alloc(sizeof(uint32_t) * n_docs));
            hipLaunchKernelGGL(update_slots_kernel, dim3((unsigned)((n + 255) / 256)), dim3(256), 0, st, d_pids.as<int64_t>(), n,
                               s->pid_offset, (int)n_docs, slot.as<uint32_t>());
        }
        CLB_TRY(len.alloc(sizeof(uint32_t) * (n_docs + 1)));
        CLB_TRY(c.doc_off.alloc(sizeof(uint32_t) * (n_docs + 1)));
        const auto lengths_kernel = staged ? change_lengths_kernel<true> : change_lengths_kernel<false>;
        hipLaunchKernelGGL(lengths_kernel, dim3((unsigned)((n_docs + 1 + 255) / 256)), dim3(256), 0, st, s->doc_off.as<uint32_t>(),
                           named.as<uint32_t>(), slot.as<uint32_t>(), stage_off.as<uint32_t>(), (int)n_docs, len.as<uint32_t>(),
                           counts.ptr());
        CLB_TRY(err.read(st));
        CLB_TRY(counts.read(st));
        if (err.value & kErrCode) return bad_codes();
        if (err.value) return fail(CLB_EBOUNDS, "a pid outside the searcher's passages");
        if (staged) CLB_TRY(check_shard_limits(n_old - (int64_t)counts.value.dropped + n_add, n_docs));
        if (counts.value.changed == 0) return CLB_OK;
        uint32_t n_rows = 0;
        CLB_TRY(exclusive_scan_u32(len.as<uint32_t>(), c.doc_off.as<uint32_t>(), (size_t)n_docs, st));
        CLB_HIP(hipMemcpyAsync(&n_rows, c.doc_off.as<uint32_t>() + n_docs, sizeof n_rows, hipMemcpyDeviceToHost, st));
        CLB_HIP(hipStreamSynchronize(st));
        c.n_docs = n_docs; c.n_emb = n_rows; c.max_doclen = counts.value.longest;
        CLB_TRY(build_live_bitmap(st, c.doc_off.as<uint32_t>(), n_docs, &c.live));

        DevBuf codes_staged, res_staged;
        if (staged) {
            CLB_TRY(codes_staged.alloc(sizeof(uint32_t) * n_add));
            CLB_TRY(res_staged.alloc(rows * n_add));
            CLB_TRY(stage_new_rows(s, codes_in.as<uint32_t>(), stage_off.as<uint32_t>(), n_add, n, residuals, on_device,
                                   codes_staged.as<uint32_t>(), res_staged.as<uint8_t>()));
        }
        CLB_TRY(alloc_padded_rows(st, c.n_emb, rows, &c.codes0, &c.residuals));
        const int64_t row_tiles = (c.n_emb + kTile - 1) / kTile;
        if (row_tiles > 0)
            with_piece(rows, [&](auto piece) {
                using Piece = decltype(piece);
                const auto rows_kernel = staged ? splice_rows_kernel<Piece, true> : splice_rows_kernel<Piece, false>;
                hipLaunchKernelGGL(rows_kernel, dim3((unsigned)std::min<int64_t>(row_tiles, 8192)), dim3(256), 0, st, s->doc_off.as<uint32_t>(),
                                   c.doc_off.as<uint32_t>(), named.as<uint32_t>(), slot.as<uint32_t>(), stage_off.as<uint32_t>(),
                                   (int)n_docs, c.n_emb, s->codes0.as<uint32_t>(), s->residuals.as<Piece>(),
                                   codes_staged.as<uint32_t>(), res_staged.as<Piece>(), (int)(rows / sizeof(Piece)),
                                   c.codes0.as<uint32_t>(), c.residuals.as<Piece>());
            });

        DevBuf pos, kept_off, kept_pid;
// ... 38 lines not shown
}

static int searcher_create_impl(int device, int64_t dim, int nbits, int64_t K, const float* centroids,
                                const float* bucket_weights, int64_t n_docs, const int64_t* doclens, int64_t n_emb,
                                const uint32_t* codes, const uint8_t* residuals, const int64_t* ivf,
                                const int64_t* ivf_lengths, int64_t pid_offset, bool big_on_device, clb_searcher** out) {
    const hipMemcpyKind big_kind = big_on_device ? hipMemcpyDeviceToDevice : hipMemcpyHostToDevice;
    if (!out) return fail(CLB_EARGUMENT, "out is null");
    *out = nullptr;
    if (dim < 8 || dim % 8 != 0) return fail(CLB_EDOMAIN, "dim should be a multiple of 8!");
    if (nbits != 1 && nbits != 2 && nbits != 4 && nbits != 8)
        return fail(CLB_EUNSUPPORTED, "the HIP codec supports nbits in {1,2,4,8} (got %d)", nbits);
    if (K < 1 || n_docs < 0 || n_emb < 0) return fail(CLB_EARGUMENT, "negative or empty sizes");
    CLB_TRY(check_shard_limits(n_emb, n_docs));
    Offsets docs, lists;
    CLB_TRY(passage_offsets(doclens, n_docs, n_emb, "passage", &docs));
    if (running_offsets(ivf_lengths, K, &lists) >= 0) return fail(CLB_EARGUMENT, "negative ivf length");
    if (lists.total != n_emb) return fail(CLB_EDIMENSION, "length(ivf) must be equal to sum(ivf_lengths)!");
    CLB_TRY(use_device(device));

    static std::atomic<uint64_t> next_serial{1};
    std::unique_ptr<clb_searcher, decltype(&clb_searcher_destroy)> owned(new clb_searcher(), clb_searcher_destroy);
    clb_searcher* s = owned.get();
    s->serial = next_serial.fetch_add(1);
    s->device = device; s->dim = dim; s->nbits = nbits; s->K = K; s->n_docs = n_docs; s->n_emb = n_emb;
    s->pid_offset = pid_offset;
    s->generic = !(dim == kDim && nbits <= 4);
    s->max_doclen = docs.longest;
    CLB_HIP(hipStreamCreateWithFlags(&s->stream, hipStreamNonBlocking));
    const hipStream_t st = s->stream;
    s->ivf_len_sorted = sorted_list_lengths(lists.off);

    const size_t rows = (size_t)(dim / 8 * nbits);
    CLB_TRY(s->centroids.alloc(sizeof(float) * dim * K));
    CLB_HIP(hipMemcpyAsync(s->centroids.p, centroids, sizeof(float) * dim * K, big_kind, st));
    CLB_TRY(upload(s->weights, bucket_weights, sizeof(float) * ((size_t)1 << nbits), st));
    CLB_TRY(alloc_padded_rows(st, n_emb, rows, &s->codes0, &s->residuals));
    CLB_HIP(hipMemcpyAsync(s->residuals.p, residuals, rows * n_emb, big_kind, st));
    CLB_TRY(upload(s->doc_off, docs.off.data(), sizeof(uint32_t) * docs.off.size(), st));
    CLB_TRY(build_live_bitmap(st, s->doc_off.as<uint32_t>(), n_docs, &s->live));
    CLB_TRY(upload(s->ivf_off, lists.off.data(), sizeof(uint32_t) * lists.off.size(), st));
    CLB_TRY(s->ivf_pid.alloc(sizeof(uint32_t) * n_emb));
    DevBuf ivf_raw;
    DevWord<int> err;
    CLB_TRY(ivf_raw.alloc(sizeof(int64_t) * n_emb));
    CLB_TRY(err.init(st));
    CLB_TRY(stage_codes(st, codes, big_kind, n_emb, K, s->codes0.as<uint32_t>(), err.ptr()));
    if (n_emb > 0) {
        CLB_HIP(hipMemcpyAsync(ivf_raw.p, ivf, sizeof(int64_t) * n_emb, big_kind, st));
        hipLaunchKernelGGL(ivf_to_pid_kernel, dim3((unsigned)((n_emb + 255) / 256)), dim3(256), 0, st, ivf_raw.as<int64_t>(),
                           s->doc_off.as<uint32_t>(), s->ivf_pid.as<uint32_t>(), n_emb, (int)n_docs, err.ptr());
        hipLaunchKernelGGL(ivf_lists_sorted_kernel, dim3((unsigned)((K + 3) / 4)), dim3(256), 0, st,
                           s->ivf_off.as<uint32_t>(), s->ivf_pid.as<uint32_t>(), (int)K, err.ptr());
    }
    CLB_TRY(err.read(st));
    if (err.value & kErrIvfId) return fail(CLB_EBOUNDS, "ivf holds embedding ids outside 1..n_emb");
    if (err.value & kErrCode) return bad_codes();
    s->ivf_sorted = !(err.value & kErrUnsortedList);

    if (s->generic) {
        s->index_bytes = resident_bytes(s);
        *out = owned.release();
        return CLB_OK;
    }
    if (n_emb > 0) {
        DevBuf codes_new, res_new;
        CLB_TRY(alloc_padded_rows(st, n_emb, rows, &codes_new, &res_new));
        CLB_TRY(order_rows_by_code(st, s->codes0.as<uint32_t>(), s->doc_off.as<uint32_t>(), n_emb, n_docs,
                                   s->residuals.as<uint8_t>(), rows, codes_new.as<uint32_t>(), res_new.as<uint8_t>()));
        swap_buf(s->codes0, codes_new); swap_buf(s->residuals, res_new);
    }
    const int64_t nel = dim * K;
    CLB_TRY(s->cent_hi.alloc(sizeof(uint16_t) * nel));
    CLB_TRY(s->cent_lo.alloc(sizeof(uint16_t) * nel));
    CLB_TRY(s->cent_f16.alloc(sizeof(uint16_t) * nel));
    hipLaunchKernelGGL(split_bf16_kernel, dim3((unsigned)((nel + 255) / 256)), dim3(256), 0, st,
                       s->centroids.as<float>(), s->cent_hi.as<uint16_t>(), s->cent_lo.as<uint16_t>(), nel);
    hipLaunchKernelGGL(to_f16_kernel, dim3((unsigned)((nel + 255) / 256)), dim3(256), 0, st,
                       s->centroids.as<float>(), s->cent_f16.as<uint16_t>(), nel);
    s->cbits = 1;
    while (((int64_t)1 << s->cbits) < K) ++s->cbits;
    s->approx_ok = approx_supported((int)dim, nbits) && s->cbits <= 20;
    IndexTables tables;
    CLB_TRY(derive_index_tables(s, s->codes0.as<uint32_t>(), s->residuals.as<uint8_t>(), n_emb, &tables));
    install_index_tables(s, tables);
    s->mode = s->approx_ok ? 1 : 0;
    *out = owned.release();
    return CLB_OK;
}

int clb_searcher_create(int device, int64_t dim, int nbits, int64_t K, const float* centroids,
                        const float* bucket_weights, int64_t n_docs, const int64_t* doclens, int64_t n_emb,
                        const uint32_t* codes, const uint8_t* residuals, const int64_t* ivf,
                        const int64_t* ivf_lengths, int64_t pid_offset, clb_searcher** out) {
    return searcher_create_impl(device, dim, nbits, K, centroids, bucket_weights, n_docs, doclens, n_emb, codes, residuals,
                                ivf, ivf_lengths, pid_offset, false, out);
}

int clb_searcher_create_device(int device, int64_t dim, int nbits, int64_t K, const float* d_centroids,
                               const float* bucket_weights, int64_t n_docs, const int64_t* doclens, int64_t n_emb,
                               const uint32_t* d_codes, const uint8_t* d_residuals, const int64_t* d_ivf,
                               const int64_t* ivf_lengths, int64_t pid_offset, clb_searcher** out) {
    return searcher_create_impl(device, dim, nbits, K, d_centroids, bucket_weights, n_docs, doclens, n_emb, d_codes,
                                d_residuals, d_ivf, ivf_lengths, pid_offset, true, out);
}

int clb_searcher_destroy(clb_searcher* s) {
    if (!s) return CLB_OK;
    (void)hipSetDevice(s->device);
    if (s->stream) {
        (void)hipStreamSynchronize(s->stream);
        for (auto& v : s->prof.pending)
            for (auto& pr : v) { (void)hipEventDestroy(pr.first); (void)hipEventDestroy(pr.second); }
        for (auto e : s->prof.pool) (void)hipEventDestroy(e);
        (void)hipStreamDestroy(s->stream);
    }
    delete s;
    return CLB_OK;
}

static int searcher_append_impl(clb_searcher* s, int64_t n_new, const int64_t* doclens, int64_t n_new_emb,
                                const uint32_t* codes, const uint8_t* residuals, bool on_device) {
    if (!s) return fail(CLB_EARGUMENT, "null searcher");
    if (n_new < 0 || n_new_emb < 0) return fail(CLB_EARGUMENT, "negative sizes");
    if ((n_new > 0 && !doclens) || (n_new_emb > 0 && (!codes || !residuals))) return fail(CLB_EARGUMENT, "null argument");
    Offsets add;
    CLB_TRY(passage_offsets(doclens, n_new, n_new_emb, "appended passage", &add));
    if (n_new == 0) return CLB_OK;
    const int64_t n_old = s->n_emb, d_old = s->n_docs;
    IndexChange c;
    c.n_docs = d_old + n_new; c.n_emb = n_old + n_new_emb; c.max_doclen = std::max<int64_t>(s->max_doclen, add.longest);
    CLB_TRY(check_shard_limits(c.n_emb, c.n_docs));
    CLB_TRY(begin_index_change(s));
    const hipStream_t st = s->stream;
    const size_t rows = (size_t)(s->dim / 8 * s->nbits);
    {
        DevBuf codes_in, new_off_d;
        DevWord<int> err;
        CLB_TRY(codes_in.alloc(sizeof(uint32_t) * n_new_emb));
        CLB_TRY(err.init(st));
        CLB_TRY(stage_codes(st, codes, on_device ? hipMemcpyDeviceToDevice : hipMemcpyHostToDevice, n_new_emb, s->K,
                            codes_in.as<uint32_t>(), err.ptr()));
        CLB_TRY(err.read(st));
        if (err.value & kErrCode) return bad_codes();

        CLB_TRY(alloc_padded_rows(st, c.n_emb, rows, &c.codes0, &c.residuals));
        CLB_TRY(c.doc_off.alloc(sizeof(uint32_t) * (c.n_docs + 1)));
        CLB_TRY(upload(new_off_d, add.off.data(), sizeof(uint32_t) * add.off.size(), st));
        CLB_HIP(hipMemcpyAsync(c.codes0.p, s->codes0.p, sizeof(uint32_t) * n_old, hipMemcpyDeviceToDevice, st));
        CLB_HIP(hipMemcpyAsync(c.residuals.p, s->residuals.p, rows * n_old, hipMemcpyDeviceToDevice, st));
        CLB_HIP(hipMemcpyAsync(c.doc_off.p, s->doc_off.p, sizeof(uint32_t) * (d_old + 1), hipMemcpyDeviceToDevice, st));
        std::vector<uint32_t> off_tail((size_t)n_new);
        for (int64_t p = 0; p < n_new; ++p) off_tail[p] = (uint32_t)(n_old + add.off[p + 1]);
        CLB_HIP(hipMemcpyAsync(c.doc_off.as<uint32_t>() + d_old + 1, off_tail.data(), sizeof(uint32_t) * n_new, hipMemcpyHostToDevice, st));
        CLB_TRY(build_live_bitmap(st, c.doc_off.as<uint32_t>(), c.n_docs, &c.live));
        if (n_new_emb > 0)
            CLB_TRY(stage_new_rows(s, codes_in.as<uint32_t>(), new_off_d.as<uint32_t>(), n_new_emb, n_new, residuals, on_device,
                                   c.codes0.as<uint32_t>() + n_old, c.residuals.as<uint8_t>() + rows * n_old));

        NewEntries e;
        CLB_TRY(sort_new_entries(s, codes_in.as<uint32_t>(), new_off_d.as<uint32_t>(), n_new, nullptr, d_old, n_new_emb, false, &e));
        CLB_TRY(merge_lists(s, s->ivf_off.as<uint32_t>(), s->ivf_pid.as<uint32_t>(), e, &c));
        CLB_HIP(hipStreamSynchronize(st));
    }
    return commit_index_change(s, c);
}

// ... 18 lines not shown

static int searcher_update_impl(clb_searcher* s, int64_t n, const int64_t* pids, const int64_t* doclens, int64_t n_new_emb,
                                const uint32_t* codes, const uint8_t* residuals, bool on_device, int64_t* n_changed) {
    if (n_changed) *n_changed = 0;
    if (!s) return fail(CLB_EARGUMENT, "null searcher");
    if (n < 0 || n_new_emb < 0) return fail(CLB_EARGUMENT, "negative sizes");
    if ((n > 0 && (!pids || !doclens)) || (n_new_emb > 0 && (!codes || !residuals))) return fail(CLB_EARGUMENT, "null argument");
    Offsets add;
    CLB_TRY(passage_offsets(doclens, n, n_new_emb, "replaced passage", &add));
    CLB_TRY(check_pid_range(s, pids, n));
    {
        std::vector<int64_t> sorted(pids, pids + n);
        std::sort(sorted.begin(), sorted.end());
        const auto twice = std::adjacent_find(sorted.begin(), sorted.end());
        if (twice != sorted.end())
            return fail(CLB_EARGUMENT, "pid %lld is named twice: an update takes one new content per passage", (long long)*twice);
    }
    if (n == 0) return CLB_OK;
    return replace_passages(s, n, pids, &add, codes, residuals, on_device, n_changed);
}
int clb_searcher_update(clb_searcher* s, int64_t n, const int64_t* pids, const int64_t* doclens, int64_t n_new_emb,
                        const uint32_t* codes, const uint8_t* residuals, int64_t* n_changed) {
    return searcher_update_impl(s, n, pids, doclens, n_new_emb, codes, residuals, false, n_changed);
}
int clb_searcher_update_device(clb_searcher* s, int64_t n, const int64_t* pids, const int64_t* doclens, int64_t n_new_emb,
                               const uint32_t* d_codes, const uint8_t* d_residuals, void* hip_stream, int64_t* n_changed) {
    (void)hip_stream;
    return searcher_update_impl(s, n, pids, doclens, n_new_emb, d_codes, d_residuals, true, n_changed);
}
int64_t clb_searcher_generation(const clb_searcher* s) { return s ? s->generation : -(int64_t)fail(CLB_EARGUMENT, "null searcher"); }
int64_t clb_searcher_num_docs(const clb_searcher* s) { return s ? s->n_docs : -(int64_t)fail(CLB_EARGUMENT, "null searcher"); }
int64_t clb_searcher_num_embeddings(const clb_searcher* s) { return s ? s->n_emb : -(int64_t)fail(CLB_EARGUMENT, "null searcher"); }

int64_t clb_searcher_device_bytes(const clb_searcher* s) {
    if (!s) return 0;
    int64_t tot = s->index_bytes;
    for (const auto& w : s->ws) {
        const DevBuf* bufs[] = {&w.Qdev, &w.cells, &w.cells_q, &w.partial, &w.sel, &w.bitmap, &w.blocksum, &w.ncand, &w.cand,
                                &w.cand_hdr, &w.scores, &w.list, &w.nlist, &w.thresh, &w.outp, &w.outs, &w.flags, &w.stats, &w.redo, &w.rowmask, &w.eps_pair, &w.tokmax, &w.tau_glob, &w.tscale, &w.rangep, &w.cells8};
        for (auto* b : bufs) tot += (int64_t)b->bytes;
    }
    return tot;
}

int clb_searcher_set_mode(clb_searcher* s, int mode) {
    if (!s) return fail(CLB_EARGUMENT, "null searcher");
    if (mode != 0 && mode != 1) return fail(CLB_EARGUMENT, "mode must be 0 (exact) or 1 (two-pass)");
    if (mode == 1 && !s->approx_ok) return fail(CLB_EUNSUPPORTED, "two-pass mode needs dim=128, nbits=2");
    s->mode = mode;
    return CLB_OK;
}
int clb_searcher_get_mode(const clb_searcher* s) { return s ? s->mode : -1; }

int clb_searcher_set_wide_select(clb_searcher* s, int on) {
    if (!s) return fail(CLB_EARGUMENT, "null searcher");
    if (on < -1 || on > 1) return fail(CLB_EARGUMENT, "wide select must be -1 (by candidate capacity), 0 (never) or 1 (always)");
    s->wide_select = on;
    return CLB_OK;
}

int clb_searcher_sync_bound_consts(clb_searcher* s, clb_comm* c) {
    if (!s || !c) return fail(CLB_EARGUMENT, "null argument");
    CLB_TRY(use_device(s->device));
    float consts[6];
    CLB_TRY(clb_searcher_get_bound_consts(s, consts));
    DevBuf d;
    CLB_TRY(upload(d, consts, sizeof consts, s->stream));
    CLB_TRY(clb_comm_all_reduce_max_f32(c, d.as<float>(), 6, s->stream));
    CLB_HIP(hipMemcpyAsync(consts, d.p, sizeof consts, hipMemcpyDeviceToHost, s->stream));
    CLB_HIP(hipStreamSynchronize(s->stream));
    return clb_searcher_set_bound_consts(s, consts);
}

int clb_searcher_set_pass1_gather(clb_searcher* s, int form) {
    if (!s) return fail(CLB_EARGUMENT, "null searcher");
    if (form < -1 || form > 1) return fail(CLB_EARGUMENT, "pass-1 gather form must be -1 (by the code statistics), 0 (VGPR) or 1 (LDS-DMA)");
    s->gather_lds = form < 0 ? default_gather_lds(s) : form;
    return CLB_OK;
}
int clb_searcher_get_pass1_gather(const clb_searcher* s, double* adjacency) {
    if (!s) return -1;
    if (adjacency) *adjacency = s->code_adjacency;
    return s->gather_lds;
}

int clb_searcher_set_score_rows(clb_searcher* s, int form) {
    if (!s) return fail(CLB_EARGUMENT, "null searcher");
    if (form < -1 || form > 1) return fail(CLB_EARGUMENT, "score rows must be -1 (default: fp16), 0 (64-byte fp16 rows) or 1 (32-byte rows of 8-bit cells)");
    if (form == 1 && !s->approx_ok) return fail(CLB_EUNSUPPORTED, "8-bit score rows need the two-pass mode (dim=128, nbits=2)");
    s->cell8 = form;
    return CLB_OK;
}
int clb_searcher_get_score_rows(const clb_searcher* s) { return s ? (cell8_rows(s) ? 1 : 0) : -1; }

int clb_searcher_set_centroid_products(clb_searcher* s, int n) {
    if (!s) return fail(CLB_EARGUMENT, "null searcher");
    if (n != -1 && n != 1 && n != 3) return fail(CLB_EARGUMENT, "centroid products must be -1 (default), 1 (one fp16 product) or 3 (bf16 split)");
    s->s1_x1 = n == 1 ? 1 : n == 3 ? 0 : -1;
    return CLB_OK;
}
int clb_searcher_get_centroid_products(const clb_searcher* s, float* max_f16_error) {
    if (!s) return -1;
    if (max_f16_error) *max_f16_error = s->dc_f16;
    return single_product_table(s) ? 1 : 3;
}

int clb_searcher_get_bound_consts(const clb_searcher* s, float* consts) {
    if (!s || !consts) return fail(CLB_EARGUMENT, "null argument");
    bound_consts_to_abi(s->approx_consts, consts);
    return CLB_OK;
}
int clb_searcher_set_bound_consts(clb_searcher* s, const float* consts) {
    if (!s || !consts) return fail(CLB_EARGUMENT, "null argument");
    for (int i = 0; i < 6; ++i)
        if (!(consts[i] >= 0.f)) return fail(CLB_EARGUMENT, "bound constants must be non-negative numbers");
    raise_bound_consts(s->approx_consts, consts);
    s->bounds_synced = true;
    return CLB_OK;
}

int clb_search_batch_device(clb_searcher* s, const float* d_Q, int64_t T, int64_t B, int64_t nprobe,
                            int64_t k, int64_t* d_out_pids, float* d_out_scores, int64_t* d_n_cand,
                            void* hip_stream) {
    return clb_search_batch_device_slot(s, 0, d_Q, T, B, nprobe, k, d_out_pids, d_out_scores, d_n_cand, hip_stream);
}

static int search_batch_device_slot_impl(clb_searcher* s, int slot, const float* d_Q, int64_t T, int64_t B, int64_t nprobe,
                                         int64_t k, const clb_filter* const* filters, int scope, const clb_grouping* grp,
                                         int64_t per_group , int64_t* d_out_pids,
                                         float* d_out_scores, int64_t* d_n_cand, void* hip_stream, PriorArg prior = {},
                                         AfterArg after = {}) {
    CLB_TRY(check_search_args(s, T, B, nprobe, k));
    Workspace* w = nullptr;
    CLB_TRY(slot_workspace(s, slot, &w));
    hipStream_t st = (hipStream_t)hip_stream;
    CLB_TRY(for_sub_batches(s, *w, T, B, nprobe, k, filters, scope, grp, per_group, prior, after.s != nullptr, [&](int64_t b0, Batch& q) -> int {
        q.dQ = d_Q + (size_t)b0 * T * s->dim;
        if (after.s) { q.d_after_s = after.s + b0; q.d_after_p = after.p + b0; }
        q.d_out_pids = per_group ? w->hit_p.as<int64_t>() : d_out_pids + (size_t)b0 * k;
        q.d_out_scores = per_group ? w->hit_s.as<float>() : d_out_scores + (size_t)b0 * k;
        q.d_hit_pids = d_out_pids + (size_t)b0 * k * per_group;
        q.d_hit_scores = d_out_scores + (size_t)b0 * k * per_group;
        q.d_n_cand = d_n_cand ? d_n_cand + b0 : nullptr;
        return run_search(s, *w, st, q);
    }));
    if (grp && !per_group && B <= kSubBatch) {
        auto& d = w->grouped_done;
        d.valid = true; d.B = B; d.k = k; d.generation = s->generation; d.grp = grp; d.stream = hip_stream;
    }
    return CLB_OK;
}

int clb_search_batch_device_slot(clb_searcher* s, int slot, const float* d_Q, int64_t T, int64_t B, int64_t nprobe,
                                 int64_t k, int64_t* d_out_pids, float* d_out_scores, int64_t* d_n_cand,
                                 void* hip_stream) {
    return search_batch_device_slot_impl(s, slot, d_Q, T, B, nprobe, k, nullptr, CLB_FILTER_CANDIDATES, nullptr, 0, d_out_pids,
                                         d_out_scores, d_n_cand, hip_stream);
}

int clb_search_batch_filtered_device_slot(clb_searcher* s, int slot, const float* d_Q, int64_t T, int64_t B, int64_t nprobe,
                                          int64_t k, const clb_filter* const* filters, int scope, int64_t* d_out_pids,
                                          float* d_out_scores, int64_t* d_n_cand, void* hip_stream) {
    return search_batch_device_slot_impl(s, slot, d_Q, T, B, nprobe, k, filters, scope, nullptr, 0, d_out_pids, d_out_scores,
                                         d_n_cand, hip_stream);
}

// ... 603 lines not shown
                                  int64_t n_lists, int64_t B, const int64_t* d_n_cand_lists, const int64_t* d_edge_gids,
                                  int64_t* d_out_pids, float* d_out_scores, int64_t* d_out_n_cand, void* hip_stream) {
    return merge_topk_grouped_launch(device, d_pids, d_scores, d_gids, k, n_lists, B, (size_t)(B * k), (size_t)(B * k),
                                     (size_t)(B * k), d_n_cand_lists, (size_t)B, d_edge_gids, (size_t)(2 * B), d_out_pids,
                                     d_out_scores, d_out_n_cand, hip_stream);
}

int64_t clb_packed_grouped_bytes(int64_t k, int64_t B) { return clb_packed_topk_bytes(k, B) + 8 * B * k + 8 * B + 16 * B; }

int clb_merge_topk_grouped_packed_device(int device, const void* d_packed, int64_t k, int64_t n_lists, int64_t B,
                                         int64_t* d_out_pids, float* d_out_scores, int64_t* d_out_n_cand, void* hip_stream) {
    if (k < 1 || B < 1) return fail(CLB_EARGUMENT, "k, n_lists and B must be >= 1");
    if (!d_packed) return fail(CLB_EARGUMENT, "d_packed is null");
    const size_t block = (size_t)clb_packed_grouped_bytes(k, B);
    const size_t at_gids = (size_t)clb_packed_topk_bytes(k, B), at_n = at_gids + (size_t)B * k * 8, at_edges = at_n + (size_t)B * 8;
    const char* base = static_cast<const char*>(d_packed);
    return merge_topk_grouped_launch(device, reinterpret_cast<const int64_t*>(base),
                                     reinterpret_cast<const float*>(base + (size_t)B * k * 8),
                                     reinterpret_cast<const int64_t*>(base + at_gids), k, n_lists, B, block / 8, block / 4, block / 8,
                                     reinterpret_cast<const int64_t*>(base + at_n), block / 8,
                                     reinterpret_cast<const int64_t*>(base + at_edges), block / 8, d_out_pids, d_out_scores,
                                     d_out_n_cand, hip_stream);
}

int clb_debug_group_tau_device(const float* d_all_top, const int64_t* d_all_gid, int64_t n_shards, int64_t B, int64_t k,
                               float* d_tau, void* hip_stream) {
    if (!d_all_top || !d_all_gid || !d_tau) return fail(CLB_EARGUMENT, "d_all_top, d_all_gid or d_tau is null");
    if (n_shards < 1 || B < 1 || k < 1) return fail(CLB_EARGUMENT, "n_shards, B and k must be >= 1");
    if (n_shards > kMaxGroupShards)
        return fail(CLB_EUNSUPPORTED, "at most %d shards, got %lld", kMaxGroupShards, (long long)n_shards);
    if (n_shards * k > INT32_MAX) return fail(CLB_EUNSUPPORTED, "n_shards * k exceeds 2^31 - 1");
    hipLaunchKernelGGL(group_global_tau_kernel, dim3((unsigned)B), dim3(1024), 0, (hipStream_t)hip_stream, d_all_top, d_all_gid,
                       (int)n_shards, (int)B, (int)k, d_tau);
    CLB_HIP(hipGetLastError());
    return CLB_OK;
}

int clb_debug_prior_tau_device(const float* d_all_top, const int64_t* d_all_gid, const float* d_all_mabs, const float* d_eps,
                               int64_t n_shards, int64_t B, int64_t k, float* d_tau_in, void* hip_stream) {
    if (!d_all_top || !d_all_mabs || !d_eps || !d_tau_in)
        return fail(CLB_EARGUMENT, "d_all_top, d_all_mabs, d_eps or d_tau_in is null");
    if (n_shards < 1 || B < 1 || k < 1) return fail(CLB_EARGUMENT, "n_shards, B and k must be >= 1");
    if (d_all_gid && n_shards > kMaxGroupShards)
        return fail(CLB_EUNSUPPORTED, "at most %d shards with group indices, got %lld", kMaxGroupShards, (long long)n_shards);
    if (n_shards * k > INT32_MAX) return fail(CLB_EUNSUPPORTED, "n_shards * k exceeds 2^31 - 1");
    hipLaunchKernelGGL(prior_global_tau_kernel, dim3((unsigned)B), dim3(1024), 0, (hipStream_t)hip_stream, d_all_top, d_all_gid,
                       d_all_mabs, (int)n_shards, (int)B, (int)k, d_eps, (const float*)nullptr, 0, ApproxConsts{},
                       (const float4*)nullptr, 0, d_tau_in);
    CLB_HIP(hipGetLastError());
    return CLB_OK;
}

int clb_merge_topk_packed_device(int device, const void* d_packed, int64_t k, int64_t n_lists, int64_t B,
                                 int64_t* d_out_pids, float* d_out_scores, void* hip_stream) {
    if (k < 1 || B < 1) return fail(CLB_EARGUMENT, "k, n_lists and B must be >= 1");
    const size_t block = (size_t)clb_packed_topk_bytes(k, B);
    const char* base = static_cast<const char*>(d_packed);
    return merge_topk_launch(device, reinterpret_cast<const int64_t*>(base),
                             reinterpret_cast<const float*>(base + (size_t)B * k * 8), k, n_lists, B, block / 8, block / 4,
                             d_out_pids, d_out_scores, hip_stream);
}

int clb_debug_scores(clb_searcher* s, const float* Q, int64_t T, int64_t nprobe, int64_t k, int64_t cap,
                     int64_t* out_pids, float* out_approx, float* out_exact, int64_t* n_out, float* tau,
                     float* eps, int64_t* n_rescore) {
    CLB_TRY(check_search_args(s, T, 1, nprobe, k));
    if (!s->approx_ok || T > 32) return fail(CLB_EUNSUPPORTED, "two-pass mode not available for this index/query");
    CLB_TRY(use_device(s->device));
    Workspace& w = s->ws[0];
    w.pending.valid = false;
    const int Bd = cell8_rows(s) ? kTeamQueries : 1;
    CLB_TRY(ensure_workspace(s, w, Bd, T, nprobe, k));
    hipStream_t st = s->stream;
    for (int c = 0; c < Bd; ++c)
        CLB_HIP(hipMemcpyAsync(w.Qdev.as<float>() + (size_t)c * T * kDim, Q, sizeof(float) * T * kDim, hipMemcpyHostToDevice, st));
    const float* dQ = w.Qdev.as<float>();
    {
        const int mode = s->mode;
        s->mode = 1;
        const int rc = run_retrieve(s, w, st, make_batch(dQ, Bd, T, nprobe, k));
        s->mode = mode;
        CLB_TRY(rc);
    }
    launch_pass1(s, w, st, dQ, dim3(8 * 32), Bd, (int)T);
    ApproxConsts ac = s->approx_consts;
    ac.dc_max = bound_dc(s, w);
    hipLaunchKernelGGL(select_margin_kernel, dim3(1), dim3(1024), 0, st, w.scores.as<float>(), w.ncand.as<int>(), dQ,
                       (int)T, (int)k, w.cand_cap, ac, w.list.as<int>(), w.nlist.as<int>(),
                       w.thresh.as<float>(), w.eps_pair.as<float>(), (const float*)nullptr, 0,
                       w.have_range ? (const float4*)w.tscale.as<float4>() : (const float4*)nullptr, w.cell8 ? 1 : 0);
    int nc = 0, nl = 0;
    float th[2];
    CLB_HIP(hipMemcpyAsync(&nc, w.ncand.p, sizeof(int), hipMemcpyDeviceToHost, st));
    CLB_HIP(hipMemcpyAsync(&nl, w.nlist.p, sizeof(int), hipMemcpyDeviceToHost, st));
    CLB_HIP(hipMemcpyAsync(th, w.thresh.p, sizeof th, hipMemcpyDeviceToHost, st));
    CLB_HIP(hipStreamSynchronize(st));
    if (nc > cap) return fail(CLB_EARGUMENT, "output capacity %lld < %d candidates", (long long)cap, nc);
    std::vector<uint32_t> c((size_t)nc);
    if (nc) {
        CLB_HIP(hipMemcpy(c.data(), w.cand.p, sizeof(uint32_t) * nc, hipMemcpyDeviceToHost));
        CLB_HIP(hipMemcpy(out_approx, w.scores.p, sizeof(float) * nc, hipMemcpyDeviceToHost));
    }
    switch (s->nbits) {
        case 2: launch_score_exact<2>(s, w, st, dQ, 1, (int)T, nullptr, nullptr, 2048); break;
        default: return fail(CLB_EUNSUPPORTED, "nbits");
    }
    CLB_HIP(hipGetLastError());
    CLB_HIP(hipStreamSynchronize(st));
    if (nc) CLB_HIP(hipMemcpy(out_exact, w.scores.p, sizeof(float) * nc, hipMemcpyDeviceToHost));
    for (int i = 0; i < nc; ++i) out_pids[i] = s->pid_offset + (int64_t)c[i] + 1;
    *n_out = nc; *tau = th[0]; *eps = th[1]; *n_rescore = nl;
    return CLB_OK;
}

int clb_profile_enable(clb_searcher* s, int on) {
    if (!s) return fail(CLB_EARGUMENT, "null searcher");
    s->prof.on = on != 0;
    s->prof.counters = on >= 2;
    return CLB_OK;
}

int clb_profile_read(clb_searcher* s, const char** names, double* total_ms, int64_t* launches, int cap) {
    if (!s) return 0;
    (void)hipSetDevice(s->device);
    (void)hipDeviceSynchronize();
    int n = 0;
    std::vector<hipEvent_t> seen;
    s->prof.chain = nullptr;
    for (int id = 0; id < KID_COUNT && n < cap; ++id) {
        for (auto& pr : s->prof.pending[id]) {
            float ms = 0.f;
            if (hipEventElapsedTime(&ms, pr.first, pr.second) == hipSuccess) {
                s->prof.total_ms[id] += ms;
                s->prof.launches[id] += 1;
            }
            seen.push_back(pr.first);
            seen.push_back(pr.second);
        }
        s->prof.pending[id].clear();
        names[n] = kKernelNames[id];
        total_ms[n] = s->prof.total_ms[id];
        launches[n] = s->prof.launches[id];
        s->prof.total_ms[id] = 0;
        s->prof.launches[id] = 0;
        ++n;
    }
    std::sort(seen.begin(), seen.end());
    seen.erase(std::unique(seen.begin(), seen.end()), seen.end());
    s->prof.pool.insert(s->prof.pool.end(), seen.begin(), seen.end());
    if (s->prof.failed) {
        s->prof.failed = false;
        (void)fail(CLB_EHIP, "HIP event creation/record failed while profiling: timings are incomplete");
        return -1;
    }
    return n;
}

int clb_last_batch_stats(clb_searcher* s, int64_t* cand_docs, int64_t* cand_embs, int64_t* rescored_docs,
                         int64_t* rescored_embs) {
    if (!s) return fail(CLB_EARGUMENT, "null searcher");
    CLB_TRY(use_device(s->device));
    CLB_HIP(hipDeviceSynchronize());
    unsigned long long h[8] = {0};
    for (auto& w : s->ws) {
        unsigned long long t[8] = {0};
        if (w.stats.p) CLB_HIP(hipMemcpy(t, w.stats.p, sizeof t, hipMemcpyDeviceToHost));
        for (int i = 0; i < 8; ++i) h[i] += t[i];
// ... 26 lines not shown
```

colbert.jl_amd/csrc/search_kernels.hpp:

```cpp
#pragma once
#include <hip/hip_fp16.h>

#include <type_traits>

#include "common.hpp"

namespace clb {

typedef float f32x16 __attribute__((ext_vector_type(16)));
typedef float f32x4 __attribute__((ext_vector_type(4)));

constexpr int kDim = 128;
constexpr int kCentTileStride = 132;
constexpr int kMaxTopK = 16384;

static __global__ __launch_bounds__(128) void centroid_scores_kernel(const float* __restrict__ C,
                                                               const float* __restrict__ Q,
                                                               float* __restrict__ cells, int K, int T,
                                                               int TT, int n_tiles) {
    extern __shared__ __attribute__((aligned(16))) float lds[];
    const int wave = threadIdx.x >> 6, lane = threadIdx.x & 63;
    const int i = lane & 31, h = lane >> 5;
    const int b = blockIdx.y / TT, tt = blockIdx.y % TT;
    const int Tpad = TT * 32;
// ... 1201 lines not shown
        }
    }
    for (int i = tid; i < n; i += 1024) {
        const int slot = lst[i];
        keys[i] = ((unsigned long long)f32_order_key(sc[slot]) << 32) | (unsigned long long)(0xffffffffu - (uint32_t)slot);
    }
    __syncthreads();
    const uint32_t* cnd = cand + (size_t)b * cand_cap;
    const int e = tid & 255, quarter = __builtin_amdgcn_readfirstlane(tid >> 8);
    const int q0 = (int)(((long long)n * quarter) >> 2), q1 = (int)(((long long)n * (quarter + 1)) >> 2);
    for (int base = g * 256; base < n; base += kRankBlocks * 256) {
        const int i = base + e;
        if (tid < 256) ranks[tid] = 0;
        __syncthreads();
        const unsigned long long mine = i < n ? keys[i] : ~0ull;
        int cnt = 0;
#pragma unroll 4
        for (int j = q0; j < q1; ++j) cnt += keys[j] > mine;
        if (cnt) atomicAdd(&ranks[e], cnt);
        __syncthreads();
        if (tid < 256 && i < n) {
            const int r = ranks[e];
            if (r < keff) {
                const uint32_t slot = 0xffffffffu - (uint32_t)(mine & 0xffffffffull);
                out_pids[(size_t)b * k + r] = pid_offset + (int64_t)cnd[slot] + 1;
                out_scores[(size_t)b * k + r] = sc[slot];
            }
        }
        __syncthreads();
    }
}

static __global__ void ivf_to_pid_kernel(const int64_t* __restrict__ ivf, const uint32_t* __restrict__ doc_off,
                                  uint32_t* __restrict__ ivf_pid, int64_t n_emb, int n_docs,
                                  int* __restrict__ err) {
    const int64_t i = (int64_t)blockIdx.x * blockDim.x + threadIdx.x;
    if (i >= n_emb) return;
    const int64_t eid = ivf[i] - 1;
    if (eid < 0 || eid >= n_emb) { atomicOr(err, 1); ivf_pid[i] = 0; return; }
    int lo = 0, hi = n_docs;
    while (hi - lo > 1) {
        const int mid = (lo + hi) >> 1;
        if ((int64_t)doc_off[mid] <= eid) lo = mid; else hi = mid;
    }
    ivf_pid[i] = (uint32_t)lo;
}

static __global__ void ivf_lists_sorted_kernel(const uint32_t* __restrict__ ivf_off, const uint32_t* __restrict__ ivf_pid,
                                               int K, int* __restrict__ unsorted) {
    const int c = blockIdx.x * 4 + (threadIdx.x >> 6), lane = threadIdx.x & 63;
    if (c >= K) return;
    const uint32_t lo = ivf_off[c], hi = ivf_off[c + 1];
    bool bad = false;
    for (uint32_t i = lo + 1 + lane; i < hi; i += 64) bad |= ivf_pid[i] < ivf_pid[i - 1];
    if (bad) atomicOr(unsorted, 4);
}

static __global__ void passage_code_keys_kernel(const uint32_t* __restrict__ codes0, const uint32_t* __restrict__ doc_off,
                                                int64_t n_emb, int n_docs, unsigned long long* __restrict__ keys,
                                                uint32_t* __restrict__ vals) {
    const int64_t e = (int64_t)blockIdx.x * blockDim.x + threadIdx.x;
    if (e >= n_emb) return;
    int lo = 0, hi = n_docs;
    while (hi - lo > 1) {
        const int mid = (lo + hi) >> 1;
        if ((int64_t)doc_off[mid] <= e) lo = mid; else hi = mid;
    }
    keys[e] = ((unsigned long long)(uint32_t)lo << 32) | codes0[e];
    vals[e] = (uint32_t)e;
}
static __global__ void permute_codes_kernel(const uint32_t* __restrict__ perm, const uint32_t* __restrict__ src,
                                            uint32_t* __restrict__ dst, int64_t n) {
    const int64_t e = (int64_t)blockIdx.x * blockDim.x + threadIdx.x;
    if (e < n) dst[e] = src[perm[e]];
}
static __global__ void permute_rows16_kernel(const uint32_t* __restrict__ perm, const uint4* __restrict__ src,
                                             uint4* __restrict__ dst, int64_t n, int pieces ) {
    const int64_t i = (int64_t)blockIdx.x * blockDim.x + threadIdx.x;
    if (i >= n * pieces) return;
    const int64_t e = i / pieces;
    const int q = (int)(i % pieces);
    dst[i] = src[(size_t)perm[e] * pieces + q];
}

static __global__ void codes_to_zero_based_kernel(uint32_t* __restrict__ codes, int64_t n, uint32_t K,
                                           int* __restrict__ err) {
    const int64_t i = (int64_t)blockIdx.x * blockDim.x + threadIdx.x;
    if (i >= n) return;
    const uint32_t c = codes[i];
    if (c < 1u || c > K) { atomicOr(err, 2); codes[i] = 0; } else codes[i] = c - 1u;
}

static __global__ void batch_stats_kernel(const uint32_t* __restrict__ cand, const int* __restrict__ ncand,
                                   const int* __restrict__ list, const int* __restrict__ nlist,
                                   const uint32_t* __restrict__ doc_off, size_t cand_cap,
                                   unsigned long long* __restrict__ stats,
                                   const unsigned long long* __restrict__ rowmask , int T) {
    const int b = blockIdx.y;
    const uint32_t* cnd = cand + (size_t)b * cand_cap;
    unsigned long long embs = 0, lembs = 0, lo_rows = 0, hi_rows = 0;
    const int n = ncand[b];
    for (int i = blockIdx.x * blockDim.x + threadIdx.x; i < n; i += gridDim.x * blockDim.x) {
        const uint32_t p = cnd[i];
        embs += doc_off[p + 1] - doc_off[p];
    }
    const int nl = list ? nlist[b] : 0;
    for (int i = blockIdx.x * blockDim.x + threadIdx.x; i < nl; i += gridDim.x * blockDim.x) {
        const uint32_t p = cnd[list[(size_t)b * cand_cap + i]];
        const uint32_t len = doc_off[p + 1] - doc_off[p];
        if (rowmask && len <= (uint32_t)kMaxMaskedRows) {
            const unsigned long long* mw = rowmask + ((size_t)b * cand_cap + i) * 8;
            lembs += __popcll(mw[0] | mw[4]) + __popcll(mw[1] | mw[5]) + __popcll(mw[2] | mw[6]) + __popcll(mw[3] | mw[7]);
            lo_rows += __popcll(mw[0]) + __popcll(mw[1]) + __popcll(mw[2]) + __popcll(mw[3]);
            hi_rows += __popcll(mw[4]) + __popcll(mw[5]) + __popcll(mw[6]) + __popcll(mw[7]);
        } else {
            lembs += len;
            if (rowmask) {
                lo_rows += len;
                hi_rows += T > 16 ? len : 0u;
            }
        }
    }
    for (int o = 32; o > 0; o >>= 1) {
        embs += __shfl_down(embs, o, 64);
        lembs += __shfl_down(lembs, o, 64);
        lo_rows += __shfl_down(lo_rows, o, 64);
        hi_rows += __shfl_down(hi_rows, o, 64);
    }
    if ((threadIdx.x & 63) == 0) {
        if (embs) atomicAdd(&stats[1], embs);
        if (lembs) atomicAdd(&stats[3], lembs);
        if (lo_rows) atomicAdd(&stats[4], lo_rows);
        if (hi_rows) atomicAdd(&stats[5], hi_rows);
    }
    if (blockIdx.x == 0 && threadIdx.x == 0) {
        atomicAdd(&stats[0], (unsigned long long)n);
        atomicAdd(&stats[2], (unsigned long long)nl);
    }
}

__device__ __forceinline__ bool rec_before(float s, int64_t p, float s2, int64_t p2) {
    const uint32_t a = f32_order_key(s), a2 = f32_order_key(s2);
    return a > a2 || (a == a2 && p < p2);
}
static __global__ __launch_bounds__(256) void merge_topk_kernel(const int64_t* __restrict__ pids,
                                                         const float* __restrict__ scores, int k, int n_lists,
                                                         int B, size_t pid_stride, size_t score_stride,
                                                         int64_t* __restrict__ out_pids,
                                                         float* __restrict__ out_scores) {
    const int b = blockIdx.y;
    const int idx = blockIdx.x * blockDim.x + threadIdx.x;
    if (idx >= n_lists * k) return;
    const int l = idx / k, i = idx % k;
    const int64_t p = pids[(size_t)l * pid_stride + (size_t)b * k + i];
    const float s = scores[(size_t)l * score_stride + (size_t)b * k + i];
    if (p <= 0) return;
    int rank = i;
    for (int l2 = 0; l2 < n_lists; ++l2) {
        if (l2 == l) continue;
        const int64_t* pl = pids + (size_t)l2 * pid_stride + (size_t)b * k;
        const float* sl = scores + (size_t)l2 * score_stride + (size_t)b * k;
        int lo = 0, hi = k;
        while (lo < hi) {
            const int mid = (lo + hi) >> 1;
            const int64_t p2 = pl[mid];
            const float s2 = sl[mid];
// ... 16 lines not shown
```

colbert.jl_amd/searcher.py:

```python
from __future__ import annotations

import ctypes as C
import os
from typing import Optional

import numpy as np

from . import storage
from ._lib import BoundsError, ColBERTError, check, colmajor, fptr, i64, lib
from .config import ColBERTConfig


_SCOPES = {"candidates": 0, "all": 1}


def _scope_code(scope) -> int:
    if scope not in _SCOPES:
        raise ColBERTError(f"scope must be 'candidates' or 'all', got {scope!r}")
    return _SCOPES[scope]


MAX_PER_GROUP = 16


# ... 303 lines not shown
        if persist and self.index_path is None:
            raise ColBERTError("persist=True needs a Searcher opened from an index_path")
        p = np.ascontiguousarray(np.asarray(pids.cpu() if hasattr(pids, "data_ptr") else pids).reshape(-1), dtype=np.int64)
        dl = np.ascontiguousarray(np.asarray(doclens.cpu() if hasattr(doclens, "data_ptr") else doclens).reshape(-1), dtype=np.int64)
        if p.size != dl.size:
            raise ColBERTError(f"one doclen per pid: {p.size} pids, {dl.size} doclens")
        n = i64(0)
        if hasattr(codes, "data_ptr"):
            st = self._check_device_rows(codes, residuals)
            check(lib().clb_searcher_update_device(self._h, i64(p.size), fptr(p), fptr(dl), i64(codes.numel()),
                                                   C.c_void_p(codes.data_ptr()), C.c_void_p(residuals.data_ptr()),
                                                   C.c_void_p(st), C.byref(n)))
            if persist:
                co, r = self._rows_to_host(codes, residuals)
        else:
            co, r = self._check_host_rows(codes, residuals)
            check(lib().clb_searcher_update(self._h, i64(p.size), fptr(p), fptr(dl), i64(co.size), fptr(co), fptr(r),
                                            C.byref(n)))
        self.num_embeddings = int(lib().clb_searcher_num_embeddings(self._h))
        if persist and n.value:
            storage.update_passages(self.index_path, p - self.pid_offset, co, r, dl)
        return int(n.value)

    def update_embeddings(self, pids, embs, doclens, persist: bool = False) -> int:
        codes, res = self._compress(embs)
        return self.update_compressed(pids, codes, res, doclens, persist=persist)

    def update_passages(self, pids, texts, persist: bool = False) -> int:
        if self.encoder is None:
            raise ColBERTError("no encoder attached: pass encoder=... or use update_embeddings(pids, embs, doclens)")
        embs, doclens = self.encoder.encode_passages(list(texts))
        return self.update_embeddings(pids, embs, doclens, persist=persist)

    def _index_codec(self):
        if self._codec is None:
            from .codec import Codec
            cent, cut = self._codec_src
            if cut is None:
                raise ColBERTError("this index carries no bucket_cutoffs: embeddings cannot be compressed with its codec "
                                   "(pass an index with 'bucket_cutoffs', or use add_compressed)")
            cut = np.asarray(cut.cpu() if hasattr(cut, "data_ptr") else cut, dtype=np.float32)
            self._codec = Codec(cent, cut, self.dim, self.nbits, device=self.device)
        return self._codec

    def _compress(self, embs):
        import torch
        codec = self._index_codec()
        if hasattr(embs, "data_ptr"):
            x = embs
        else:
            e = colmajor(embs, np.float32)
            if e.ndim != 2 or e.shape[0] != self.dim:
                raise ColBERTError(f"embs must be (dim={self.dim}, n)")
            x = torch.from_numpy(np.ascontiguousarray(e.T)).to(torch.device("cuda", self.device))
        return codec.compress_device(x)

    def add_embeddings(self, embs, doclens, persist: bool = False) -> range:
        codes, res = self._compress(embs)
        return self.add_compressed(codes, res, doclens, persist=persist)

    def add_passages(self, texts, persist: bool = False) -> range:
        if self.encoder is None:
            raise ColBERTError("no encoder attached: pass encoder=... or use add_embeddings(embs, doclens)")
        embs, doclens = self.encoder.encode_passages(list(texts))
        return self.add_embeddings(embs, doclens, persist=persist)

    @property
    def device_bytes(self) -> int:
        return int(lib().clb_searcher_device_bytes(self._h))

    def set_mode(self, mode: int):
        check(lib().clb_searcher_set_mode(self._h, C.c_int(mode)))

    def set_wide_select(self, on: int):
        check(lib().clb_searcher_set_wide_select(self._h, C.c_int(on)))

    def set_pass1_gather(self, form: int):
        check(lib().clb_searcher_set_pass1_gather(self._h, C.c_int(form)))

    @property
    def pass1_gather(self):
        adj = C.c_double(0)
        return int(lib().clb_searcher_get_pass1_gather(self._h, C.byref(adj))), adj.value

    def set_score_rows(self, form: int):
        check(lib().clb_searcher_set_score_rows(self._h, C.c_int(form)))

    @property
    def score_rows(self) -> int:
        return int(lib().clb_searcher_get_score_rows(self._h))

    def set_centroid_products(self, n: int):
        check(lib().clb_searcher_set_centroid_products(self._h, C.c_int(n)))

    @property
    def centroid_products(self):
        dc = C.c_float(0)
        return int(lib().clb_searcher_get_centroid_products(self._h, C.byref(dc))), dc.value

    @property
    def mode(self) -> int:
        return int(lib().clb_searcher_get_mode(self._h))

    @property
    def bound_consts(self) -> np.ndarray:
        out = np.zeros(6, dtype=np.float32)
        check(lib().clb_searcher_get_bound_consts(self._h, fptr(out)))
        return out

    def raise_bound_consts(self, consts):
        c = np.ascontiguousarray(consts, dtype=np.float32)
        assert c.shape == (6,)
        check(lib().clb_searcher_set_bound_consts(self._h, fptr(c)))

    def make_filter(self, pids=None, mask=None) -> PassageFilter:
        if (pids is None) == (mask is None):
            raise ColBERTError("make_filter takes exactly one of pids= and mask=")
        h = C.c_void_p()
        if pids is not None:
            p = np.ascontiguousarray(np.asarray(pids).reshape(-1), dtype=np.int64)
            check(lib().clb_filter_create_pids(self._h, fptr(p), i64(p.size), C.byref(h)))
        else:
            m = np.asarray(mask)
            if m.dtype != np.bool_ or m.shape != (self.num_docs,):
                raise ColBERTError(f"mask must be a boolean array of num_docs={self.num_docs} entries")
            words = np.ascontiguousarray(np.packbits(m, bitorder="little"))
            words = np.concatenate([words, np.zeros(-words.size % 4, np.uint8)]).view("<u4")
            check(lib().clb_filter_create_bitmap(self._h, fptr(words), i64(words.size), C.byref(h)))
        return PassageFilter(self, h, lib().clb_filter_count(h))

    def _filter_handles(self, filters, B: int):
        if isinstance(filters, PassageFilter):
            filters = [filters] * B
        filters = list(filters)
        if len(filters) != B:
            raise ColBERTError(f"filters must be one PassageFilter or a sequence of B={B} entries (None = unfiltered)")
        arr = (C.c_void_p * B)()
        for j, f in enumerate(filters):
            if f is None:
                continue
            if not isinstance(f, PassageFilter) or not f._h:
                raise ColBERTError(f"filters[{j}] is not an open PassageFilter")
            arr[j] = f._h.value
        return arr

    def make_grouping(self, group_ids=None, group_lens=None) -> PassageGrouping:
        if (group_ids is None) == (group_lens is None):
            raise ColBERTError("make_grouping takes exactly one of group_ids= and group_lens=")
        if group_lens is not None:
            lens = np.asarray(group_lens)
            if lens.ndim != 1 or lens.dtype.kind not in "iu" or (lens.size and int(lens.min()) < 0) or int(lens.sum()) != self.num_docs:
                raise ColBERTError(f"group_lens must be non-negative integers summing to num_docs={self.num_docs}")
            ids = np.repeat(np.arange(lens.size, dtype=np.int64), lens.astype(np.int64))
        else:
            ids = np.asarray(group_ids)
            if ids.ndim != 1 or ids.dtype.kind not in "iu":
                raise ColBERTError("group_ids must be a vector of integers, one per passage")
            ids = np.ascontiguousarray(ids, dtype=np.int64).copy()
        h = C.c_void_p()
        check(lib().clb_grouping_create(self._h, fptr(ids), i64(ids.size), C.byref(h)))
        return PassageGrouping(self, h, lib().clb_grouping_count(h), ids)

    def _grouping_handle(self, grouping):
        if not isinstance(grouping, PassageGrouping) or not grouping._h:
            raise ColBERTError("grouping is not an open PassageGrouping")
        return grouping._h
# ... 338 lines not shown
```

include/colbert_hip.h:

```cpp
#ifndef COLBERT_HIP_H
#define COLBERT_HIP_H
#include <stdint.h>
#ifdef __cplusplus
extern "C" {
#endif

#define CLB_OK 0
#define CLB_EDIMENSION 1
#define CLB_EDOMAIN 2
#define CLB_EBOUNDS 3
#define CLB_EARGUMENT 4
#define CLB_EHIP 10
#define CLB_EUNSUPPORTED 11
#define CLB_ENOMEM 12

typedef struct clb_searcher clb_searcher;

const char* clb_version(void);
const char* clb_last_error(void);
int clb_device_count(void);
int clb_measure_copy_rate(int device, int64_t bytes, int reps, double* gb_per_s);
int clb_measure_read_rate(int device, int64_t bytes, int reps, double* gb_per_s);

int clb_searcher_create(int device, int64_t dim, int nbits, int64_t K,
                        const float* centroids , const float* bucket_weights ,
                        int64_t n_docs, const int64_t* doclens, int64_t n_emb,
                        const uint32_t* codes ,
                        const uint8_t* residuals ,
                        const int64_t* ivf ,
                        const int64_t* ivf_lengths , int64_t pid_offset,
                        clb_searcher** out);
int clb_searcher_create_device(int device, int64_t dim, int nbits, int64_t K, const float* d_centroids,
                               const float* bucket_weights, int64_t n_docs, const int64_t* doclens, int64_t n_emb,
                               const uint32_t* d_codes, const uint8_t* d_residuals, const int64_t* d_ivf,
                               const int64_t* ivf_lengths, int64_t pid_offset, clb_searcher** out);
int clb_searcher_destroy(clb_searcher* s);
int clb_searcher_append(clb_searcher* s, int64_t n_new, const int64_t* doclens, int64_t n_new_emb, const uint32_t* codes,
                        const uint8_t* residuals);
int clb_searcher_append_device(clb_searcher* s, int64_t n_new, const int64_t* doclens, int64_t n_new_emb,
                               const uint32_t* d_codes, const uint8_t* d_residuals, void* hip_stream);
int clb_searcher_remove(clb_searcher* s, const int64_t* pids, int64_t n, int64_t* n_removed);
int clb_searcher_update(clb_searcher* s, int64_t n, const int64_t* pids, const int64_t* doclens, int64_t n_new_emb,
                        const uint32_t* codes, const uint8_t* residuals, int64_t* n_changed);
int clb_searcher_update_device(clb_searcher* s, int64_t n, const int64_t* pids, const int64_t* doclens, int64_t n_new_emb,
                               const uint32_t* d_codes, const uint8_t* d_residuals, void* hip_stream, int64_t* n_changed);
int64_t clb_searcher_generation(const clb_searcher* s);
int64_t clb_searcher_num_docs(const clb_searcher* s);
int64_t clb_searcher_num_embeddings(const clb_searcher* s);
int64_t clb_searcher_device_bytes(const clb_searcher* s);

int clb_search(clb_searcher* s, const float* Q, int64_t T, int64_t nprobe, int64_t k,
               int64_t* out_pids, float* out_scores, int64_t* n_cand);
int clb_search_batch(clb_searcher* s, const float* Q, int64_t T, int64_t B, int64_t nprobe, int64_t k,
                     int pad_short, int64_t* out_pids, float* out_scores, int64_t* n_cand);
int clb_search_batch_device(clb_searcher* s, const float* d_Q, int64_t T, int64_t B, int64_t nprobe,
                            int64_t k, int64_t* d_out_pids, float* d_out_scores, int64_t* d_n_cand,
                            void* hip_stream);
int clb_search_batch_device_slot(clb_searcher* s, int slot, const float* d_Q, int64_t T, int64_t B, int64_t nprobe,
                                 int64_t k, int64_t* d_out_pids, float* d_out_scores, int64_t* d_n_cand,
                                 void* hip_stream);
int clb_search_shard_phase1(clb_searcher* s, const float* d_Q, int64_t T, int64_t B, int64_t nprobe, int64_t k,
                            float* d_local_top, void* hip_stream);
int clb_search_shard_phase2(clb_searcher* s, const float* d_Q, int64_t T, int64_t B, int64_t nprobe, int64_t k,
                            const float* d_all_top, int64_t n_shards, int64_t* d_out_pids, float* d_out_scores,
                            int64_t* d_n_cand, void* hip_stream);
int clb_search_shard_phase1_slot(clb_searcher* s, int slot, const float* d_Q, int64_t T, int64_t B, int64_t nprobe,
                                 int64_t k, float* d_local_top, void* hip_stream);
int clb_search_shard_phase2_slot(clb_searcher* s, int slot, const float* d_Q, int64_t T, int64_t B, int64_t nprobe,
                                 int64_t k, const float* d_all_top, int64_t n_shards, int64_t* d_out_pids,
                                 float* d_out_scores, int64_t* d_n_cand, void* hip_stream);
int clb_searcher_set_mode(clb_searcher* s, int mode);
int clb_searcher_get_mode(const clb_searcher* s);
int clb_searcher_set_wide_select(clb_searcher* s, int on);
int clb_searcher_set_pass1_gather(clb_searcher* s, int form);
int clb_searcher_get_pass1_gather(const clb_searcher* s, double* adjacency);
int clb_searcher_set_score_rows(clb_searcher* s, int form);
int clb_searcher_get_score_rows(const clb_searcher* s);
int clb_searcher_set_centroid_products(clb_searcher* s, int n);
int clb_searcher_get_centroid_products(const clb_searcher* s, float* max_f16_error);
int clb_searcher_get_bound_consts(const clb_searcher* s, float* consts );
int clb_searcher_set_bound_consts(clb_searcher* s, const float* consts );

typedef struct clb_filter clb_filter;
int clb_filter_create_pids(clb_searcher* s, const int64_t* pids, int64_t n, clb_filter** out);
int clb_filter_create_pids_global(clb_searcher* s, const int64_t* pids, int64_t n, clb_filter** out, int64_t* n_inside);
int clb_filter_create_bitmap(clb_searcher* s, const uint32_t* words, int64_t n_words, clb_filter** out);
int64_t clb_filter_count(const clb_filter* f);
int clb_filter_destroy(clb_filter* f);
enum { CLB_FILTER_CANDIDATES = 0, CLB_FILTER_ALL = 1 };
int clb_search_batch_filtered(clb_searcher* s, const float* Q, int64_t T, int64_t B, int64_t nprobe, int64_t k,
                              const clb_filter* const* filters, int scope, int64_t* out_pids, float* out_scores,
                              int64_t* n_cand);
int clb_search_batch_filtered_device_slot(clb_searcher* s, int slot, const float* d_Q, int64_t T, int64_t B, int64_t nprobe,
                                          int64_t k, const clb_filter* const* filters, int scope, int64_t* d_out_pids,
                                          float* d_out_scores, int64_t* d_n_cand, void* hip_stream);
int clb_search_shard_phase1_filtered_slot(clb_searcher* s, int slot, const float* d_Q, int64_t T, int64_t B, int64_t nprobe,
                                          int64_t k, const clb_filter* const* filters, int scope, float* d_local_top,
                                          void* hip_stream);

typedef struct clb_grouping clb_grouping;
int clb_grouping_create(clb_searcher* s, const int64_t* group_ids, int64_t n, clb_grouping** out);
int64_t clb_grouping_count(const clb_grouping* g);
int clb_grouping_destroy(clb_grouping* g);
int clb_search_batch_grouped(clb_searcher* s, const float* Q, int64_t T, int64_t B, int64_t nprobe, int64_t k,
                             const clb_filter* const* filters, int scope, const clb_grouping* grouping, int pad_short,
                             int64_t* out_pids, float* out_scores, int64_t* n_cand);
int clb_search_batch_grouped_device_slot(clb_searcher* s, int slot, const float* d_Q, int64_t T, int64_t B, int64_t nprobe,
                                         int64_t k, const clb_filter* const* filters, int scope, const clb_grouping* grouping,
                                         int64_t* d_out_pids, float* d_out_scores, int64_t* d_n_cand, void* hip_stream);

enum { CLB_MAX_PER_GROUP = 16 };
int clb_search_batch_grouped_hits(clb_searcher* s, const float* Q, int64_t T, int64_t B, int64_t nprobe, int64_t k,
                                  const clb_filter* const* filters, int scope, const clb_grouping* grouping, int64_t per_group,
                                  int pad_short, int64_t* out_pids, float* out_scores, int64_t* n_cand);
int clb_search_batch_grouped_hits_device_slot(clb_searcher* s, int slot, const float* d_Q, int64_t T, int64_t B, int64_t nprobe,
                                              int64_t k, const clb_filter* const* filters, int scope,
                                              const clb_grouping* grouping, int64_t per_group, int64_t* d_out_pids,
                                              float* d_out_scores, int64_t* d_n_cand, void* hip_stream);

typedef struct clb_prior clb_prior;
int clb_prior_create(clb_searcher* s, const float* values, int64_t n, clb_prior** out);
int clb_prior_create_device(clb_searcher* s, const float* d_values, int64_t n, clb_prior** out);
float clb_prior_max_abs(const clb_prior* p);
int clb_prior_destroy(clb_prior* p);
int clb_search_batch_prior(clb_searcher* s, const float* Q, int64_t T, int64_t B, int64_t nprobe, int64_t k,
                           const clb_filter* const* filters, int scope, const clb_grouping* grouping, const clb_prior* prior,
                           float weight, int pad_short, int64_t* out_pids, float* out_scores, int64_t* n_cand);
int clb_search_batch_prior_device_slot(clb_searcher* s, int slot, const float* d_Q, int64_t T, int64_t B, int64_t nprobe,
                                       int64_t k, const clb_filter* const* filters, int scope, const clb_grouping* grouping,
                                       const clb_prior* prior, float weight, int64_t* d_out_pids, float* d_out_scores,
                                       int64_t* d_n_cand, void* hip_stream);

int clb_search_batch_after(clb_searcher* s, const float* Q, int64_t T, int64_t B, int64_t nprobe, int64_t k,
                           const clb_filter* const* filters, int scope, const float* after_scores ,
                           const int64_t* after_pids , int64_t* out_pids, float* out_scores, int64_t* n_cand);
int clb_search_batch_after_device_slot(clb_searcher* s, int slot, const float* d_Q, int64_t T, int64_t B, int64_t nprobe,
                                       int64_t k, const clb_filter* const* filters, int scope, const float* d_after_scores,
                                       const int64_t* d_after_pids, int64_t* d_out_pids, float* d_out_scores,
                                       int64_t* d_n_cand, void* hip_stream);

int clb_search_shard_phase1_grouped_slot(clb_searcher* s, int slot, const float* d_Q, int64_t T, int64_t B, int64_t nprobe,
                                         int64_t k, const clb_filter* const* filters, int scope, const clb_grouping* grouping,
                                         int64_t group_base, float* d_local_top, int64_t* d_local_gid, void* hip_stream);
int clb_search_shard_phase2_grouped_slot(clb_searcher* s, int slot, const float* d_Q, int64_t T, int64_t B, int64_t nprobe,
                                         int64_t k, const float* d_all_top, const int64_t* d_all_gid, int64_t n_shards,
                                         const clb_grouping* grouping, int64_t group_base, int64_t* d_out_pids,
                                         float* d_out_scores, int64_t* d_out_gids, int64_t* d_n_cand, int64_t* d_edge_gids,
                                         void* hip_stream);
int clb_search_result_groups_slot(clb_searcher* s, int slot, const clb_grouping* grouping, int64_t group_base,
                                  const int64_t* d_pids, int64_t B, int64_t k, int64_t* d_out_gids, int64_t* d_edge_gids,
                                  void* hip_stream);
int clb_debug_group_tau_device(const float* d_all_top, const int64_t* d_all_gid, int64_t n_shards, int64_t B, int64_t k,
                               float* d_tau, void* hip_stream);

int clb_search_shard_phase1_prior_slot(clb_searcher* s, int slot, const float* d_Q, int64_t T, int64_t B, int64_t nprobe,
                                       int64_t k, const clb_filter* const* filters, int scope, const clb_grouping* grouping,
                                       int64_t group_base, const clb_prior* prior, float weight, float* d_local_top,
                                       int64_t* d_local_gid, float* d_local_mabs, void* hip_stream);
// ... 165 lines not shown
```

Baseline: 31220.

## Add optional two-band pass-1 scoring split by centroid code half

Adds an opt-in mode that splits each passage's rows into two bands by whether their centroid code is below K/2. Pass 1 then runs as two kernel launches, the first writing per-token band maxima to a new buffer and the second merging them in. A per-document split table is built at index load. Separately, the tokmax and score stores in pass 1 become nontemporal, which applies in the default path too. The banding aims to shrink the centroid LUT working set per launch, at the cost of an extra launch and extra global traffic for the band maxima.

```diff
diff --git a/colbert.jl_amd/csrc/approx_kernels.hpp b/colbert.jl_amd/csrc/approx_kernels.hpp
--- a/colbert.jl_amd/csrc/approx_kernels.hpp
+++ b/colbert.jl_amd/csrc/approx_kernels.hpp
@@ -875,14 +875,16 @@
 constexpr int kApproxThreads = 768;
 constexpr int kApproxLdsLut = 256 * 256;
 
-template <bool ROWS, int GL = 0, bool CELL8 = false>
+template <bool ROWS, int GL = 0, bool CELL8 = false, int PH = 0>
 static __global__ __launch_bounds__(kApproxThreads, kApproxThreads / 256) void score_approx32_kernel(
     const float* __restrict__ weights, const uint32_t* __restrict__ codeinv, const uint8_t* __restrict__ residuals,
     int cbits, float inv_lo, float inv_step, const float* __restrict__ Q, const uint32_t* __restrict__ cells16,
     const uint2* __restrict__ cand_hdr, const int* __restrict__ ncand, float* __restrict__ scores, int K, int T,
     int B, size_t cand_cap, uint16_t* __restrict__ tokmax, const int* __restrict__ list,
     const int* __restrict__ nlist, const float* __restrict__ eps_pair, unsigned long long* __restrict__ rowmask,
-    const float4* __restrict__ tscale = nullptr) {
+    const float4* __restrict__ tscale = nullptr, const uint32_t* __restrict__ cand = nullptr,
+    const uint32_t* __restrict__ band_split = nullptr, float* __restrict__ bandmax = nullptr) {
+    static_assert(PH == 0 || (!ROWS && !CELL8), "two bands: pass 1 over fp16 rows only");
     const uint32_t cmask = (1u << cbits) - 1u;
     const int lane = threadIdx.x & 63;
     const int r = lane & 31, h = lane >> 5;
@@ -961,6 +963,8 @@
         const uint32_t h16 = 16u * (uint32_t)h;
         float* out = scores + (size_t)b * cand_cap;
         uint16_t* tmax = tokmax + (size_t)b * cand_cap * 32 + r;
+        float* bmx = PH ? bandmax + (size_t)b * cand_cap * 32 + r : nullptr;
+        const uint32_t* cnd = PH ? cand + (size_t)b * cand_cap : nullptr;
         const int* lst = ROWS ? list + (size_t)b * cand_cap : nullptr;
         unsigned long long* rmask = ROWS ? rowmask + (size_t)b * cand_cap * 8 : nullptr;
         const float window = ROWS ? 2.f * eps_pair[b] : 0.f;
@@ -974,7 +978,12 @@
         const int jl = j0 + lane;
         int slot_l = jl < j_end ? jl : j0;
         if (ROWS) slot_l = lst[slot_l];
-        const uint2 hv = hdr[slot_l];
+        uint2 hv = hdr[slot_l];
+        if (PH) {
+            const uint32_t sp_ = min(band_split[cnd[slot_l]], hv.y);
+            if (PH == 1 && hv.y) hv.y = max(sp_, 1u);
+            if (PH == 2 && hv.y) { const uint32_t st_ = min(sp_, hv.y - 1u); hv.x += st_; hv.y -= st_; }
+        }
         const int nd = j_end - j0 < 64 ? j_end - j0 : 64;
         int it_k = 0;
         uint32_t it_off = __builtin_amdgcn_readlane(hv.x, 0);
@@ -982,9 +991,10 @@
         int it_slot = __builtin_amdgcn_readlane(slot_l, 0);
         int it_base = 0;
 
-#define CLB_STAGE_A(RB, CV, PM, TAG)                                                                    \
+#define CLB_STAGE_A(RB, CV, PM, PF, TAG)                                                                \
     {                                                                                                       \
         const bool live = it_k < nd;                                                                        \
+        const int slot_h_ = live ? it_slot : 0;      \
         const uint32_t e0 = live ? it_off + (uint32_t)it_base : 0u;                                         \
         const int left = live ? it_len - it_base : kStepRows;                                               \
         const int rows = left < kStepRows ? left : kStepRows;                                               \
@@ -1026,6 +1036,8 @@
             }                                                                                               \
         } else it_base += kStepRows;                                                                        \
         if (ROWS) PM = tmax[(size_t)slot_t * 32];               \
+         \
+        if (PH == 2) PF = __builtin_nontemporal_load(bmx + (size_t)(h ? slot_t : slot_h_) * 32);            \
         const uint32_t q8_ = 8u * (uint32_t)TAG.g;                                                          \
                        \
         const uint32_t rr = (uint32_t)r < q8_ ? min((uint32_t)r, (uint32_t)(TAG.rowsh - 1))                 \
@@ -1070,7 +1082,9 @@
             X0 = *reinterpret_cast<const u32x4*>(myring + (SLOT) * 1024 + gl8_x);                           \
         } else if (GL) {                                                                                    \
              \
-            asm volatile("s_waitcnt vmcnt(4)" ::: "memory");                                                \
+             \
+            if (PH == 2) asm volatile("s_waitcnt vmcnt(5)" ::: "memory");                                   \
+            else asm volatile("s_waitcnt vmcnt(4)" ::: "memory");                                           \
             X0 = *reinterpret_cast<const u32x4*>(myring + (SLOT) * 2048 + gl_x0);                           \
             X1 = *reinterpret_cast<const u32x4*>(myring + (SLOT) * 2048 + gl_x1);                           \
         }                                                                                                   \
@@ -1102,12 +1116,15 @@
                 __builtin_bit_cast(f16x8, u32x4{tl[2 * s_].x, tl[2 * s_].y, tl[2 * s_ + 1].x, tl[2 * s_ + 1].y}), \
                 __builtin_bit_cast(f16x8, qb[s_]), ACC, 0, 0, 0);                                           \
     }
-#define CLB_PASSAGE_END(MX, J, LAST)                                                                        \
+#define CLB_PASSAGE_END(MX, J, LAST, PF, HALF)                                                              \
     {                                                                                                       \
-        float m_ = max_lane_halves(MX);                                                                     \
+         \
+        float m_ = max_lane_halves(PH == 2 && h == (HALF) ? fmaxf(MX, PF) : (MX));                          \
         if (CELL8) m_ *= stp;                         \
         const float sum = sum_lanes_0_31(r < T ? m_ : 0.f);                      \
-        if ((J) >= 0) {                                                                                \
+        if (PH == 1) {                         \
+            if ((J) >= 0 && h == 0) __builtin_nontemporal_store(m_, bmx + (size_t)(J) * 32);                \
+        } else if ((J) >= 0) {                                                                              \
                    \
             const int p_ = ((J) - j0) & 15;                                                                 \
             if (h == 0) *reinterpret_cast<uint16_t*>(mystage + p_ * 64 + 2 * r) = (uint16_t)f32_to_f16_floor(m_); \
@@ -1117,14 +1134,16 @@
                 __builtin_amdgcn_wave_barrier();                                                            \
                 const u32x4 tk_ = *reinterpret_cast<const u32x4*>(mystage + 16 * lane);                     \
                 const float sc_ = *reinterpret_cast<const float*>(mystage + 1024 + 4 * (lane & 15));         \
+                 \
+                 \
                 if (lane < 4 * (p_ + 1))                                                                    \
-                    *reinterpret_cast<u32x4*>(reinterpret_cast<unsigned char*>(tokmax + ((size_t)b * cand_cap + jb_) * 32) + 16 * lane) = tk_; \
-                if (lane <= p_) out[jb_ + lane] = sc_;                                                      \
+                    __builtin_nontemporal_store(tk_, reinterpret_cast<u32x4*>(reinterpret_cast<unsigned char*>(tokmax + ((size_t)b * cand_cap + jb_) * 32) + 16 * lane)); \
+                if (lane <= p_) __builtin_nontemporal_store(sc_, out + jb_ + lane);                         \
                 __builtin_amdgcn_wave_barrier();                                                            \
             }                                                                                               \
         }                                                                                                   \
     }
-#define CLB_STAGE_E(ACC, PM, TAG)                                                                     \
+#define CLB_STAGE_E(ACC, PM, PF, TAG)                                                                   \
     {                                                                                                       \
         f32x4 iq[4];                                                                                        \
         _Pragma("unroll") for (int q = 0; q < 4; ++q)                                                       \
@@ -1179,7 +1198,7 @@
                 const float q2_ = fmaxf(fmaxf(fmaxf(v[8], v[9]), v[10]), v[11]);                            \
                 const float q3_ = fmaxf(fmaxf(fmaxf(v[12], v[13]), v[14]), v[15]);                          \
                 const float mh_ = fmaxf(fmaxf(mx, q0_), fmaxf(TAG.g > 1 ? q1_ : kNegInf, TAG.g > 2 ? q2_ : kNegInf)); \
-                CLB_PASSAGE_END(mh_, TAG.jh, 1);                                                            \
+                CLB_PASSAGE_END(mh_, TAG.jh, 1, PF, 0);                                                          \
                 mx = fmaxf(fmaxf(TAG.g > 1 ? kNegInf : q1_, TAG.g > 2 ? kNegInf : q2_), q3_);               \
             } else {                                                                                        \
             float m01 = fmaxf(fmaxf(v[0], v[1]), v[2]);                                                     \
@@ -1192,7 +1211,7 @@
             mx = fmaxf(fmaxf(mx, m01), m67);                                                                \
             }                                                                                               \
             if (TAG.last) {                                                                                 \
-                CLB_PASSAGE_END(mx, TAG.j, TAG.last);                                                       \
+                CLB_PASSAGE_END(mx, TAG.j, TAG.last, PF, 1);                                                     \
                 mx = kNegInf;                                                                               \
             }                                                                                               \
         }                                                                                                   \
@@ -1202,24 +1221,25 @@
         u32x4 rb0, rb1, rb2, xa0, xa1, xa2, xb0, xb1, xb2;
         uint32_t cv0, cv1, cv2, cw0, cw1, cw2;
         uint16_t pm0 = 0, pm1 = 0, pm2 = 0;
+        float pf0 = 0.f, pf1 = 0.f, pf2 = 0.f;
         StepTag t0, t1, t2;
         f32x16 acc0;
-        CLB_STAGE_A(rb0, cv0, pm0, t0);
-        CLB_STAGE_A(rb1, cv1, pm1, t1);
+        CLB_STAGE_A(rb0, cv0, pm0, pf0, t0);
+        CLB_STAGE_A(rb1, cv1, pm1, pf1, t1);
         CLB_STAGE_G(cv0, xa0, xb0, 0); cw0 = cv0;
         while (t0.j >= 0) {
-            CLB_STAGE_A(rb2, cv2, pm2, t2);
+            CLB_STAGE_A(rb2, cv2, pm2, pf2, t2);
             CLB_STAGE_G(cv1, xa1, xb1, 1); cw1 = cv1;
             CLB_STAGE_CM(rb0, cw0, xa0, xb0, 0, acc0);
-            CLB_STAGE_E(acc0, pm0, t0);
-            CLB_STAGE_A(rb0, cv0, pm0, t0);
+            CLB_STAGE_E(acc0, pm0, pf0, t0);
+            CLB_STAGE_A(rb0, cv0, pm0, pf0, t0);
             CLB_STAGE_G(cv2, xa2, xb2, 2); cw2 = cv2;
             CLB_STAGE_CM(rb1, cw1, xa1, xb1, 1, acc0);
-            CLB_STAGE_E(acc0, pm1, t1);
-            CLB_STAGE_A(rb1, cv1, pm1, t1);
+            CLB_STAGE_E(acc0, pm1, pf1, t1);
+            CLB_STAGE_A(rb1, cv1, pm1, pf1, t1);
             CLB_STAGE_G(cv0, xa0, xb0, 0); cw0 = cv0;
             CLB_STAGE_CM(rb2, cw2, xa2, xb2, 2, acc0);
-            CLB_STAGE_E(acc0, pm2, t2);
+            CLB_STAGE_E(acc0, pm2, pf2, t2);
         }
         }
 #undef CLB_STAGE_A
diff --git a/colbert.jl_amd/csrc/search.hip b/colbert.jl_amd/csrc/search.hip
--- a/colbert.jl_amd/csrc/search.hip
+++ b/colbert.jl_amd/csrc/search.hip
@@ -96,6 +96,7 @@
     struct { bool valid = false; int64_t B = 0, k = 0, generation = 0; const clb_grouping* grp = nullptr; void* stream = nullptr; } grouped_done;
     DevBuf Qdev, cells, cells_q, partial, sel, bitmap, blocksum, ncand, cand, cand_hdr, scores, list, nlist, thresh,
         outp, outs, flags, stats, redo, rowmask, eps_pair, tokmax, tau_glob, wsel, bounds, tscale, rangep, cells8;
+    DevBuf bandmax;
     bool grouped = false;
     DevBuf grp_list, grp_n, grp_list2, grp_n2, grp_tau;
     int64_t mcap = 0;
@@ -131,12 +132,14 @@
     DevBuf ivf_off;
     DevBuf ivf_pid;
     DevBuf codeinv;
+    DevBuf band_split;
     int cbits = 0;
     float inv_lo = 0.f, inv_step = 0.f;
     DevBuf cent_hi, cent_lo;
     DevBuf cent_f16;
     float dc_f16 = 0.f;
     int s1_x1 = -1;
+    int bands = -1;
     int gather_lds = 0;
     double code_adjacency = 0.0;
     int cell8 = -1;
@@ -217,6 +220,8 @@
 }
 
 inline int default_gather_lds(const clb_searcher* s) { return s->code_adjacency < 0.2 && s->K * 64 > ((int64_t)4 << 20); }
+
+inline bool two_bands(const clb_searcher* s) { return s->approx_ok && s->band_split.p && s->bands == 2; }
 
 void allow_large_topk_lds() {
     allow_dynamic_lds(reinterpret_cast<const void*>(topk_kernel), (int)(sizeof(unsigned long long) * kMaxTopK));
@@ -291,6 +296,7 @@
         CLB_TRY(w.rowmask.ensure(sizeof(unsigned long long) * 8 * B * w.cand_cap));
         CLB_TRY(w.eps_pair.ensure(sizeof(float) * B));
         CLB_TRY(w.tokmax.ensure(sizeof(uint16_t) * 32 * B * w.cand_cap));
+        if (two_bands(s)) CLB_TRY(w.bandmax.ensure(sizeof(float) * 32 * B * w.cand_cap));
     }
     if (grouped || w.grouped) {
         CLB_TRY(w.grp_list.ensure(sizeof(int) * B * w.cand_cap));
@@ -720,7 +726,20 @@
 
 constexpr size_t kWideSelectCap = 131072;
 
-void launch_pass1(clb_searcher* s, Workspace& w, hipStream_t st, const float* dQ, dim3 grid, int B, int T) {
+int launch_pass1(clb_searcher* s, Workspace& w, hipStream_t st, const float* dQ, dim3 grid, int B, int T) {
+    if (!w.cell8 && two_bands(s)) {
+        if (w.bandmax.bytes < sizeof(float) * 32 * B * w.cand_cap) return fail(CLB_EHIP, "two-band pass 1: the slot holds no room for part 0's maxima");
+        auto part0 = s->gather_lds ? score_approx32_kernel<false, 1, false, 1> : score_approx32_kernel<false, 0, false, 1>;
+        auto part1 = s->gather_lds ? score_approx32_kernel<false, 1, false, 2> : score_approx32_kernel<false, 0, false, 2>;
+        for (auto kern : {part0, part1})
+            hipLaunchKernelGGL(kern, grid, dim3(kApproxThreads), 0, st, s->weights.as<float>(), s->codeinv.as<uint32_t>(),
+                               s->residuals.as<uint8_t>(), s->cbits, s->inv_lo, s->inv_step, dQ, w.cells_q.as<uint32_t>(),
+                               w.cand_hdr.as<uint2>(), w.ncand.as<int>(), w.scores.as<float>(), (int)s->K, T, B, w.cand_cap,
+                               w.tokmax.as<uint16_t>(), (const int*)nullptr, (const int*)nullptr, (const float*)nullptr,
+                               (unsigned long long*)nullptr, (const float4*)nullptr, (const uint32_t*)w.cand.as<uint32_t>(),
+                               (const uint32_t*)s->band_split.as<uint32_t>(), w.bandmax.as<float>());
+        return CLB_OK;
+    }
     auto kern = w.cell8 ? (s->gather_lds ? score_approx32_kernel<false, 1, true> : score_approx32_kernel<false, 0, true>)
                         : (s->gather_lds ? score_approx32_kernel<false, 1, false> : score_approx32_kernel<false, 0, false>);
     hipLaunchKernelGGL(kern, grid, dim3(kApproxThreads), 0, st, s->weights.as<float>(),
@@ -728,7 +747,8 @@
                        w.cell8 ? w.cells8.as<uint32_t>() : w.cells_q.as<uint32_t>(), w.cand_hdr.as<uint2>(), w.ncand.as<int>(),
                        w.scores.as<float>(), (int)s->K, T, B, w.cand_cap, w.tokmax.as<uint16_t>(), (const int*)nullptr,
                        (const int*)nullptr, (const float*)nullptr, (unsigned long long*)nullptr,
-                       (const float4*)w.tscale.as<float4>());
+                       (const float4*)w.tscale.as<float4>(), (const uint32_t*)nullptr, (const uint32_t*)nullptr, (float*)nullptr);
+    return CLB_OK;
 }
 inline float bound_dc(const clb_searcher* s, const Workspace& w) {
     return (w.x1_table || (s->bounds_synced && s->s1_x1 != 0 && s->cent_f16.p)) ? s->dc_f16 : 0.f;
@@ -802,7 +822,7 @@
                 const double est_cand = 0.5 * T * q.nprobe * (double)s->n_emb / (double)std::max<int64_t>(1, s->K);
                 const int gxq = est_cand < 6000.0 ? std::max(8, 256 / B) : 0;
                 const dim3 approx_grid = gxq > 0 && B > 1 ? dim3(gxq, B) : dim3(8 * kWgPerGroup);
-                launch_pass1(s, w, st, dQ, approx_grid, B, T);
+                CLB_TRY(launch_pass1(s, w, st, dQ, approx_grid, B, T));
             }
             if (q.prior && phase == 0) {
                 Timed t(s, KID_SELECT, st);
@@ -872,7 +892,8 @@
                            s->codeinv.as<uint32_t>(), s->residuals.as<uint8_t>(), s->cbits, s->inv_lo, s->inv_step, dQ,
                            w.cell8 ? w.cells8.as<uint32_t>() : w.cells_q.as<uint32_t>(), w.cand_hdr.as<uint2>(), w.ncand.as<int>(),
                            w.scores.as<float>(), (int)s->K, T, B, w.cand_cap, w.tokmax.as<uint16_t>(), list, nlist,
-                           w.eps_pair.as<float>(), w.rowmask.as<unsigned long long>(), (const float4*)w.tscale.as<float4>());
+                           w.eps_pair.as<float>(), w.rowmask.as<unsigned long long>(), (const float4*)w.tscale.as<float4>(),
+                           (const uint32_t*)nullptr, (const uint32_t*)nullptr, (float*)nullptr);
     }
     {
         Timed t(s, KID_SCORE_EXACT, st);
@@ -1112,17 +1133,27 @@
 
 int64_t resident_bytes(const clb_searcher* s) {
     return (int64_t)(s->centroids.bytes + s->weights.bytes + s->codes0.bytes + s->residuals.bytes + s->doc_off.bytes +
-                     s->ivf_off.bytes + s->ivf_pid.bytes + s->codeinv.bytes + s->live.bytes);
+                     s->ivf_off.bytes + s->ivf_pid.bytes + s->codeinv.bytes + s->live.bytes + s->band_split.bytes);
 }
 
 struct IndexTables {
     double code_adjacency = 0.0;
     ApproxConsts consts{};
     float inv_lo = 0.f, inv_step = 0.f;
-    DevBuf codeinv;
+    DevBuf codeinv, band_split;
 };
 
-int derive_index_tables(const clb_searcher* s, const uint32_t* codes0, const uint8_t* residuals, int64_t n_emb, IndexTables* t) {
+int build_band_split(hipStream_t st, const uint32_t* codes0, const uint32_t* doc_off, int64_t n_docs, uint32_t below, DevBuf* out) {
+    CLB_TRY(out->ensure(sizeof(uint32_t) * (size_t)std::max<int64_t>(n_docs, 1)));
+    if (n_docs > 0)
+        hipLaunchKernelGGL(band_split_kernel, dim3((unsigned)((n_docs + 255) / 256)), dim3(256), 0, st, codes0, doc_off, n_docs, below,
+                           out->as<uint32_t>());
+    CLB_HIP(hipGetLastError());
+    return CLB_OK;
+}
+
+int derive_index_tables(const clb_searcher* s, const uint32_t* codes0, const uint8_t* residuals, int64_t n_emb,
+                        const uint32_t* doc_off, int64_t n_docs, IndexTables* t) {
     {
         DevWord<unsigned long long> adj;
         const int64_t n_sample = std::min<int64_t>(n_emb, (int64_t)1 << 24);
@@ -1135,6 +1166,7 @@
     if (s->approx_ok) {
         CLB_TRY(t->codeinv.alloc(sizeof(uint32_t) * (n_emb + kStepRows)));
         CLB_HIP(hipMemsetAsync(t->codeinv.p, 0, t->codeinv.bytes, s->stream));
+        CLB_TRY(build_band_split(s->stream, codes0, doc_off, n_docs, (uint32_t)(s->K / 2), &t->band_split));
     }
     return build_approx_tables(s->stream, s->centroids.as<float>(), s->weights.as<float>(), codes0, residuals, n_emb, (int)s->K,
                                s->approx_ok ? t->codeinv.as<uint32_t>() : nullptr, s->cbits, 1 << s->nbits, &t->consts,
@@ -1154,6 +1186,7 @@
     s->code_adjacency = t.code_adjacency;
     s->gather_lds = default_gather_lds(s);
     swap_buf(s->codeinv, t.codeinv);
+    swap_buf(s->band_split, t.band_split);
     s->inv_lo = t.inv_lo; s->inv_step = t.inv_step;
     float old[6];
     bound_consts_to_abi(s->approx_consts, old);
@@ -1291,7 +1324,8 @@
     if ((int64_t)c.h_ivf_off[s->K] != c.n_emb)
         return fail(CLB_EHIP, "the changed inverted lists hold %lld entries, expected %lld", (long long)c.h_ivf_off[s->K],
                     (long long)c.n_emb);
-    if (!s->generic) CLB_TRY(derive_index_tables(s, c.codes0.as<uint32_t>(), c.residuals.as<uint8_t>(), c.n_emb, &c.tables));
+    if (!s->generic) CLB_TRY(derive_index_tables(s, c.codes0.as<uint32_t>(), c.residuals.as<uint8_t>(), c.n_emb, c.doc_off.as<uint32_t>(), c.n_docs,
+                                                  &c.tables));
     CLB_HIP(hipStreamSynchronize(st));
     CLB_HIP(hipGetLastError());
 
@@ -1496,7 +1530,7 @@
     while (((int64_t)1 << s->cbits) < K) ++s->cbits;
     s->approx_ok = approx_supported((int)dim, nbits) && s->cbits <= 20;
     IndexTables tables;
-    CLB_TRY(derive_index_tables(s, s->codes0.as<uint32_t>(), s->residuals.as<uint8_t>(), n_emb, &tables));
+    CLB_TRY(derive_index_tables(s, s->codes0.as<uint32_t>(), s->residuals.as<uint8_t>(), n_emb, s->doc_off.as<uint32_t>(), n_docs, &tables));
     install_index_tables(s, tables);
     s->mode = s->approx_ok ? 1 : 0;
     *out = owned.release();
@@ -1681,6 +1715,30 @@
     if (!s) return -1;
     if (adjacency) *adjacency = s->code_adjacency;
     return s->gather_lds;
+}
+
+static void resize_workspaces(clb_searcher* s) {
+    for (auto& w : s->ws) { w.Bcap = 0; w.pending.valid = false; }
+}
+int clb_searcher_set_pass1_bands(clb_searcher* s, int bands) {
+    if (!s) return fail(CLB_EARGUMENT, "null searcher");
+    if (bands != -1 && bands != 1 && bands != 2) return fail(CLB_EARGUMENT, "pass-1 bands must be -1 (default: one), 1 or 2");
+    if (bands == 2 && !s->approx_ok) return fail(CLB_EUNSUPPORTED, "two-band pass 1 needs the two-pass mode (dim=128, nbits=2)");
+    s->bands = bands;
+    resize_workspaces(s);
+    return CLB_OK;
+}
+int clb_searcher_get_pass1_bands(const clb_searcher* s) { return s ? (two_bands(s) ? 2 : 1) : -1; }
+int clb_searcher_debug_band_split(clb_searcher* s, int where) {
+    if (!s) return fail(CLB_EARGUMENT, "null searcher");
+    if (where < -1 || where > 1) return fail(CLB_EARGUMENT, "band split must be 0 (at code K / 2), -1 (every row in part 1) or 1 (every row in part 0)");
+    if (!s->band_split.p) return fail(CLB_EUNSUPPORTED, "two-band pass 1 needs the two-pass mode (dim=128, nbits=2)");
+    CLB_TRY(use_device(s->device));
+    CLB_HIP(hipDeviceSynchronize());
+    const uint32_t below = where < 0 ? 0u : where > 0 ? 0xffffffffu : (uint32_t)(s->K / 2);
+    CLB_TRY(build_band_split(s->stream, s->codes0.as<uint32_t>(), s->doc_off.as<uint32_t>(), s->n_docs, below, &s->band_split));
+    CLB_HIP(hipStreamSynchronize(s->stream));
+    return CLB_OK;
 }
 
 int clb_searcher_set_score_rows(clb_searcher* s, int form) {
@@ -2450,7 +2508,7 @@
         s->mode = mode;
         CLB_TRY(rc);
     }
-    launch_pass1(s, w, st, dQ, dim3(8 * 32), Bd, (int)T);
+    CLB_TRY(launch_pass1(s, w, st, dQ, dim3(8 * 32), Bd, (int)T));
     ApproxConsts ac = s->approx_consts;
     ac.dc_max = bound_dc(s, w);
     hipLaunchKernelGGL(select_margin_kernel, dim3(1), dim3(1024), 0, st, w.scores.as<float>(), w.ncand.as<int>(), dQ,
diff --git a/colbert.jl_amd/csrc/search_kernels.hpp b/colbert.jl_amd/csrc/search_kernels.hpp
--- a/colbert.jl_amd/csrc/search_kernels.hpp
+++ b/colbert.jl_amd/csrc/search_kernels.hpp
@@ -1307,6 +1307,14 @@
     const int q = (int)(i % pieces);
     dst[i] = src[(size_t)perm[e] * pieces + q];
 }
+static __global__ void band_split_kernel(const uint32_t* __restrict__ codes0, const uint32_t* __restrict__ doc_off, int64_t n_docs,
+                                         uint32_t below, uint32_t* __restrict__ band_split) {
+    const int64_t p = (int64_t)blockIdx.x * blockDim.x + threadIdx.x;
+    if (p >= n_docs) return;
+    uint32_t n = 0;
+    for (uint32_t e = doc_off[p], end = doc_off[p + 1]; e < end; ++e) n += codes0[e] < below;
+    band_split[p] = n;
+}
 
 static __global__ void codes_to_zero_based_kernel(uint32_t* __restrict__ codes, int64_t n, uint32_t K,
                                            int* __restrict__ err) {
diff --git a/colbert.jl_amd/searcher.py b/colbert.jl_amd/searcher.py
--- a/colbert.jl_amd/searcher.py
+++ b/colbert.jl_amd/searcher.py
@@ -409,6 +409,16 @@
     def pass1_gather(self):
         adj = C.c_double(0)
         return int(lib().clb_searcher_get_pass1_gather(self._h, C.byref(adj))), adj.value
+
+    def set_pass1_bands(self, bands: int):
+        check(lib().clb_searcher_set_pass1_bands(self._h, C.c_int(bands)))
+
+    @property
+    def pass1_bands(self) -> int:
+        return int(lib().clb_searcher_get_pass1_bands(self._h))
+
+    def debug_band_split(self, where: int):
+        check(lib().clb_searcher_debug_band_split(self._h, C.c_int(where)))
 
     def set_score_rows(self, form: int):
         check(lib().clb_searcher_set_score_rows(self._h, C.c_int(form)))
diff --git a/include/colbert_hip.h b/include/colbert_hip.h
--- a/include/colbert_hip.h
+++ b/include/colbert_hip.h
@@ -74,6 +74,9 @@
 int clb_searcher_set_wide_select(clb_searcher* s, int on);
 int clb_searcher_set_pass1_gather(clb_searcher* s, int form);
 int clb_searcher_get_pass1_gather(const clb_searcher* s, double* adjacency);
+int clb_searcher_set_pass1_bands(clb_searcher* s, int bands);
+int clb_searcher_get_pass1_bands(const clb_searcher* s);
+int clb_searcher_debug_band_split(clb_searcher* s, int where);
 int clb_searcher_set_score_rows(clb_searcher* s, int form);
 int clb_searcher_get_score_rows(const clb_searcher* s);
 int clb_searcher_set_centroid_products(clb_searcher* s, int n);
```

Result: no change. 31430 (median of 2 runs) (+0.7%).
